# hamaadshah/gan_deeplearning4j

Hardware: NVIDIA H100
Metric: images/sec (full G+D step) (higher is better)
Workload: dtype bf16

## Files before the change

gan_deeplearning4j_b200/_lib.py:

```python
from __future__ import annotations

import ctypes as C
import os

_HERE = os.path.dirname(os.path.abspath(__file__))
LIB_PATH = os.path.join(_HERE, "lib", "libb200gan.so")
NAME_LEN = 64


class B200GanError(RuntimeError):
    def __init__(self, code, msg):
        super().__init__(f"libb200gan error {code}: {msg}")
        self.code = code


class LayerDesc(C.Structure):
    _fields_ = [("type", C.c_int32), ("name", C.c_char * NAME_LEN), ("n_in", C.c_int32), ("n_out", C.c_int32),
                ("k_h", C.c_int32), ("k_w", C.c_int32), ("s_h", C.c_int32), ("s_w", C.c_int32), ("p_h", C.c_int32), ("p_w", C.c_int32),
                ("has_bias", C.c_int32), ("act", C.c_int32), ("act_alpha", C.c_float), ("updater", C.c_int32),
                ("lr", C.c_float), ("beta1", C.c_float), ("beta2", C.c_float), ("eps", C.c_float), ("l2", C.c_float),
                ("bn_decay", C.c_float), ("bn_eps", C.c_float), ("pre_h", C.c_int32), ("pre_w", C.c_int32), ("pre_c", C.c_int32),
                ("loss", C.c_int32), ("frozen", C.c_int32)]


class NetConfig(C.Structure):
    _fields_ = [("in_h", C.c_int32), ("in_w", C.c_int32), ("in_c", C.c_int32), ("max_batch", C.c_int32), ("precision", C.c_int32),
                ("grad_clip", C.c_float), ("xent_clip_eps", C.c_float), ("bn_groups", C.c_int32), ("seed", C.c_uint64)]


class GanConfig(C.Structure):
    _fields_ = [("fake_bn_train", C.c_int32), ("use_cuda_graph", C.c_int32)]


class LrSchedule(C.Structure):
    _fields_ = [("kind", C.c_int32), ("type", C.c_int32), ("initial", C.c_double), ("gamma", C.c_double), ("power", C.c_double),
                ("step", C.c_double), ("decay_rate", C.c_double), ("n_map", C.c_int32), ("map_keys", C.POINTER(C.c_int32)),
                ("map_values", C.POINTER(C.c_double))]


class Constraint(C.Structure):
    _fields_ = [("kind", C.c_int32), ("dims_mask", C.c_int32), ("max_norm", C.c_double), ("min_norm", C.c_double), ("rate", C.c_double)]


class ConvGeom(C.Structure):
    _fields_ = [(k, C.c_int32) for k in ("n", "h", "w", "c", "oh", "ow", "o", "kh", "kw", "sh", "sw", "ph", "pw")]


class TestConvOpts(C.Structure):
    _fields_ = [("epi", C.c_int32), ("act", C.c_int32), ("alpha", C.c_float), ("bias", C.POINTER(C.c_float)), ("scale", C.POINTER(C.c_float)),
                ("groups", C.c_int32), ("aux", C.POINTER(C.c_float)), ("aux2", C.POINTER(C.c_float)), ("stats", C.POINTER(C.c_double)), ("kernel", C.c_char * 64),
                ("bn", C.c_int32), ("max_ctas", C.c_int32), ("poison", C.c_int32), ("w_mn", C.c_int32), ("per_tap", C.c_int32), ("slab", C.c_int32),
                ("defer", C.c_int32), ("db", C.POINTER(C.c_float)), ("param_offset", C.c_int32), ("splits", C.c_int32)]


class EwReduceJob(C.Structure):
    _fields_ = [("n", C.c_int64), ("stride", C.c_int64), ("src_off", C.c_int64), ("dst_off", C.c_int64), ("splits", C.c_int32), ("wide", C.c_int32)]


class TestEwOpts(C.Structure):
    _fields_ = [("op", C.c_int32), ("n", C.c_int64), ("rows", C.c_int32), ("cols", C.c_int32), ("groups", C.c_int32), ("splits", C.c_int32),
                ("stride", C.c_int64)] + [(k, C.c_int32) for k in ("N", "H", "W", "C", "KH", "KW", "SH", "SW", "act")] + [
                ("alpha", C.c_float), ("clip_eps", C.c_float), ("offset", C.c_int32), ("in_place", C.c_int32), ("accumulate", C.c_int32),
                ("poison", C.c_int32), ("n_jobs", C.c_int32), ("jobs", C.POINTER(EwReduceJob)), ("n_seg", C.c_int32),
                ("seg_off", C.POINTER(C.c_int64)), ("seg_len", C.POINTER(C.c_int64)), ("seg_coef", C.POINTER(C.c_float)), ("sumsq", C.c_double),
                ("kernel", C.c_char * 64), ("loss", C.c_int32)]


class TestPoolOpts(C.Structure):
    _fields_ = [("op", C.c_int32), ("pool", C.c_int32), ("pnorm", C.c_float)] + [
                (k, C.c_int32) for k in ("N", "H", "W", "C", "KH", "KW", "SH", "SW", "PH", "PW", "offset", "poison")] + [
                ("kernel", C.c_char * 64), ("splits", C.c_int32)]


_vp, _i32, _i64, _fp = C.c_void_p, C.c_int32, C.c_int64, C.POINTER(C.c_float)
_pvp = C.POINTER(C.c_void_p)

PROTOTYPES = {
    "b2g_version": (_i32, []),
    "b2g_ctx_create": (_i32, [_i32, _pvp]),
    "b2g_ctx_destroy": (_i32, [_vp]),
    "b2g_last_error": (C.c_char_p, []),
    "b2g_sync": (_i32, [_vp]),
    "b2g_launch_count": (_i32, [_vp, C.POINTER(C.c_uint64)]),
    "b2g_timer_start": (_i32, [_vp]),
    "b2g_timer_stop_ms": (_i32, [_vp, _fp]),
    "b2g_flush_l2": (_i32, [_vp]),
    "b2g_device_info": (_i32, [_vp, C.POINTER(_i32), C.POINTER(_i32), C.POINTER(_i32), C.POINTER(C.c_uint64)]),
    "b2g_net_create": (_i32, [_vp, C.POINTER(NetConfig), C.POINTER(LayerDesc), _i32, _pvp]),
    "b2g_net_destroy": (_i32, [_vp]),
    "b2g_net_num_params": (_i32, [_vp, C.POINTER(_i64)]),
    "b2g_net_output_size": (_i32, [_vp, C.POINTER(_i64)]),
    "b2g_net_layer_output_size": (_i32, [_vp, _i32, C.POINTER(_i64)]),
    "b2g_net_set_param": (_i32, [_vp, C.c_char_p, C.c_char_p, _fp, _i64]),
    "b2g_net_get_param": (_i32, [_vp, C.c_char_p, C.c_char_p, _fp, _i64]),
    "b2g_net_get_params": (_i32, [_vp, _fp, _i64]),
    "b2g_net_set_params": (_i32, [_vp, _fp, _i64]),
    "b2g_net_get_gradients": (_i32, [_vp, _fp, _i64]),
    "b2g_net_updater_state_size": (_i32, [_vp, C.POINTER(_i64)]),
    "b2g_net_get_updater_state": (_i32, [_vp, _fp, _i64]),
    "b2g_net_set_updater_state": (_i32, [_vp, _fp, _i64]),
    "b2g_net_output": (_i32, [_vp, _fp, _i32, _i32, _fp]),
    "b2g_net_get_activation": (_i32, [_vp, _i32, _i32, _fp]),
    "b2g_net_compute_gradient_and_score": (_i32, [_vp, _fp, _fp, _i32, _fp]),
    "b2g_net_get_input_gradient": (_i32, [_vp, _i32, _fp]),
    "b2g_net_fit": (_i32, [_vp, _fp, _fp, _i32, _fp]),
    "b2g_net_get_iteration": (_i32, [_vp, C.POINTER(_i64)]),
    "b2g_net_set_iteration": (_i32, [_vp, _i64]),
    "b2g_net_get_dropout_pass": (_i32, [_vp, C.POINTER(_i64)]),
    "b2g_net_set_dropout_pass": (_i32, [_vp, _i64]),
    "b2g_net_set_gradient_normalization": (_i32, [_vp, _i32, C.c_float]),
    "b2g_net_set_lr_schedule": (_i32, [_vp, C.c_char_p, C.POINTER(LrSchedule)]),
    "b2g_net_set_constraints": (_i32, [_vp, C.c_char_p, C.c_char_p, C.POINTER(Constraint), _i32]),
    "b2g_net_apply_constraints": (_i32, [_vp]),
    "b2g_net_get_learning_rate": (_i32, [_vp, C.c_char_p, _fp]),
    "b2g_net_set_dropout_schedule": (_i32, [_vp, C.c_char_p, C.POINTER(LrSchedule)]),
    "b2g_net_get_dropout_value": (_i32, [_vp, C.c_char_p, _fp]),
    "b2g_net_get_epoch": (_i32, [_vp, C.POINTER(_i64)]),
    "b2g_net_set_epoch": (_i32, [_vp, _i64]),
    "b2g_net_simt_gemm_calls": (_i32, [_vp, C.POINTER(C.c_uint64)]),
    "b2g_gan_create": (_i32, [_vp, _vp, C.POINTER(GanConfig), _pvp]),
    "b2g_gan_destroy": (_i32, [_vp]),
    "b2g_gan_step": (_i32, [_vp, _fp, _fp, _fp, _fp, _fp, _fp, _i32, _fp]),
    "b2g_gan_upload": (_i32, [_vp, _fp, _fp, _fp, _fp, _fp, _fp, _i32]),
    "b2g_gan_step_resident": (_i32, [_vp, _i32]),
    "b2g_gan_read_losses": (_i32, [_vp, _fp]),
    "b2g_gan_last_step_ms": (_i32, [_vp, _fp]),
    "b2g_comm_unique_id": (_i32, [_vp]),
    "b2g_ctx_comm_init": (_i32, [_vp, _i32, _i32, _vp]),
    "b2g_ctx_comm_destroy": (_i32, [_vp]),
    "b2g_net_set_grad_allreduce": (_i32, [_vp, _i32]),
    "b2g_net_average_parameters": (_i32, [_vp]),
    "b2g_net_set_sync_bn": (_i32, [_vp, _i32]),
    "b2g_net_set_grad_payload_bf16": (_i32, [_vp, _i32]),
    "b2g_net_enable_p2p_allreduce": (_i32, [_vp, C.POINTER(C.c_int32)]),
    "b2g_ctx_allreduce_test": (_i32, [_vp, _fp, _i64]),
    "b2g_test_conv": (_i32, [_vp, _i32, _i32, _i32, C.POINTER(ConvGeom), _fp, _fp, _fp, _i32, _fp]),
    "b2g_test_hbm_kernels": (_i32, [_vp, _i32, _i32, _i32, _fp]),
    "b2g_test_conv_ex": (_i32, [_vp, _i32, _i32, _i32, C.POINTER(ConvGeom), _fp, _fp, _fp, _i32, _fp, C.POINTER(TestConvOpts)]),
    "b2g_test_bn": (_i32, [_vp, _i32, _i32, _i32, _i32, _i32, _fp, _fp, _fp, _fp, _fp, _fp, _i32, C.c_float, C.c_float, C.c_float,
                           _i32, _fp, _fp, _fp, _fp, _fp, _fp, _fp, _fp]),
    "b2g_test_net_shadow": (_i32, [_vp, _i32, _i32, _fp, _i64]),
    "b2g_test_dropout": (_i32, [_vp, _i32, C.c_uint64, _i32, _i32, _i64, _i32, _i32, _i32, _i32, C.c_float, _fp, _fp, _fp, _fp]),
    "b2g_test_dropout_kind": (_i32, [_vp, _i32, _i32, C.c_uint64, _i32, _i32, _i64, _i32, _i32, _i32, _i32, C.c_float, _fp, _fp, _fp, _fp]),
    "b2g_test_ew": (_i32, [_vp, _i32, C.POINTER(TestEwOpts), _fp, _fp, _fp, _fp, _fp]),
    "b2g_test_pool": (_i32, [_vp, _i32, C.POINTER(TestPoolOpts), _fp, _fp, _fp, _fp, _fp]),
}

_lib = None


def load():
    global _lib
    if _lib is not None:
        return _lib
    if not os.path.exists(LIB_PATH):
        raise B200GanError(-7, f"{LIB_PATH} is missing: build it with `make` (nvcc, sm_90a). There is no CPU fallback.")
    lib = C.CDLL(LIB_PATH, mode=C.RTLD_GLOBAL)
    for name, (res, args) in PROTOTYPES.items():
        fn = getattr(lib, name)
        fn.restype, fn.argtypes = res, args
    _lib = lib
    return lib


def check(code):
    if code != 0:
        raise B200GanError(code, load().b2g_last_error().decode(errors="replace"))
```

gan_deeplearning4j_b200/csrc/engine.cu:

```cuda
#include <cuda_runtime.h>
#include <dlfcn.h>
#include <math.h>
#include <stdarg.h>
#include <stdio.h>
#include <stdlib.h>
#include <string.h>

#include <algorithm>
#include <string>
#include <vector>

#include "../../include/b200gan.h"
#include "kernels.h"

using namespace b2g;

static thread_local char g_err[1024] = "";
static int32_t fail(int32_t code, const char* fmt, ...) {
  va_list ap; va_start(ap, fmt); vsnprintf(g_err, sizeof(g_err), fmt, ap); va_end(ap); return code;
}
#define CU(call) do { cudaError_t e_ = (call); if (e_ != cudaSuccess) return fail(B2G_ERR_CUDA, "%s:%d %s -> %s", __FILE__, __LINE__, #call, cudaGetErrorString(e_)); } while (0)
#define B2(call) do { int32_t r_ = (call); if (r_ != 0) return r_; } while (0)
#define CHECK_KERNELS() CU(cudaGetLastError())

// ... 1553 lines not shown
  if (!n) return fail(B2G_ERR_ARG, "null"); CU(cudaSetDevice(n->ctx->device));
  b2g_net::LayerSched ls; B2(parse_schedule(s, &ls));
  if (layer) { int li = 0; B2(find_dropout_layer(n, layer, &li)); B2(upload_dropout_schedule(n, n->L[li], ls)); }
  else for (auto& l : n->L) if (l.d.type == B2G_LAYER_DROPOUT && !l.d.frozen) B2(upload_dropout_schedule(n, l, ls));
  ++n->settings_gen;
  return 0;
}
extern "C" int32_t b2g_net_get_dropout_value(b2g_net* n, const char* layer, float* out) {
  if (!n || !layer || !out) return fail(B2G_ERR_ARG, "null"); CU(cudaSetDevice(n->ctx->device));
  int li = 0; B2(find_dropout_layer(n, layer, &li));
  const LayerRT& l = n->L[li];
  k_noise_value(l.d.act, l.d.act_alpha, noise_sched(n, l, nullptr, nullptr), n->lr_out, n->ctx->stream); CHECK_KERNELS();
  CU(cudaMemcpyAsync(out, n->lr_out, sizeof(float), cudaMemcpyDeviceToHost, n->ctx->stream)); CU(cudaStreamSynchronize(n->ctx->stream));
  return 0;
}
extern "C" int32_t b2g_net_get_epoch(b2g_net* n, int64_t* out) {
  if (!n || !out) return fail(B2G_ERR_ARG, "null"); CU(cudaSetDevice(n->ctx->device));
  int64_t v = 0; CU(cudaMemcpyAsync(&v, n->epoch_dev, sizeof(v), cudaMemcpyDeviceToHost, n->ctx->stream)); CU(cudaStreamSynchronize(n->ctx->stream)); *out = v; return 0;
}
extern "C" int32_t b2g_net_set_epoch(b2g_net* n, int64_t epoch) {
  if (!n || epoch < 0) return fail(B2G_ERR_ARG, "bad epoch"); CU(cudaSetDevice(n->ctx->device));
  CU(cudaMemcpyAsync(n->epoch_dev, &epoch, sizeof(epoch), cudaMemcpyHostToDevice, n->ctx->stream)); CU(cudaStreamSynchronize(n->ctx->stream)); return 0;
}
extern "C" int32_t b2g_net_simt_gemm_calls(b2g_net* n, uint64_t* out) { if (!n || !out) return fail(B2G_ERR_ARG, "null"); *out = n->simt_gemm_calls; return 0; }

extern "C" int32_t b2g_comm_unique_id(void* id128) { if (!id128) return fail(B2G_ERR_ARG, "null"); B2(nccl_load()); NcclId id; NC(g_nccl.uid(&id)); memcpy(id128, &id, sizeof(id)); return 0; }
extern "C" int32_t b2g_ctx_comm_init(b2g_ctx* c, int32_t world, int32_t rank, const void* id128) {
  if (!c || !id128 || world < 1 || rank < 0 || rank >= world) return fail(B2G_ERR_ARG, "bad communicator arguments");
  B2(nccl_load()); CU(cudaSetDevice(c->device));
  NcclId id; memcpy(&id, id128, sizeof(id));
  NC(g_nccl.init(&c->comm, world, id, rank)); c->world = world; c->rank = rank; return 0;
}
extern "C" int32_t b2g_ctx_comm_destroy(b2g_ctx* c) { if (c && c->comm) { g_nccl.destroy(c->comm); c->comm = nullptr; c->world = 1; c->rank = 0; } return 0; }
extern "C" int32_t b2g_net_set_grad_allreduce(b2g_net* n, int32_t enabled) { if (!n) return fail(B2G_ERR_ARG, "null"); n->grad_allreduce = enabled != 0; return 0; }
extern "C" int32_t b2g_net_set_sync_bn(b2g_net* n, int32_t enabled) { if (!n) return fail(B2G_ERR_ARG, "null"); if (enabled && n->prec != PREC_BF16) return fail(B2G_ERR_UNSUPPORTED, "sync_bn rides on the fused BatchNorm path (BF16 nets)"); n->sync_bn = enabled != 0; return 0; }
extern "C" int32_t b2g_net_set_grad_payload_bf16(b2g_net* n, int32_t enabled) {
  if (!n) return fail(B2G_ERR_ARG, "null"); CU(cudaSetDevice(n->ctx->device));
  if (enabled && !n->ar_buf) B2(dalloc(n, &n->ar_buf, sizeof(__nv_bfloat16) * (size_t)n->n_params));
  n->ar_bf16 = enabled != 0; return 0;
}
extern "C" int32_t b2g_net_enable_p2p_allreduce(b2g_net* n, int32_t* enabled) {
  if (!n) return fail(B2G_ERR_ARG, "null"); b2g_ctx* c = n->ctx; CU(cudaSetDevice(c->device)); if (enabled) *enabled = 0;
  if (!c->comm || c->world < 2) return 0;
  if (c->world > 8 || !g_nccl.ag) return 0;
  cudaStream_t s = c->stream;
  if (!c->p2p_flags) { CU(cudaMalloc(&c->p2p_flags, 16 * sizeof(unsigned))); CU(cudaMalloc(&c->p2p_state, 2 * sizeof(unsigned)));
                       CU(cudaMemsetAsync(c->p2p_flags, 0, 16 * sizeof(unsigned), s)); CU(cudaMemsetAsync(c->p2p_state, 0, 2 * sizeof(unsigned), s)); CU(cudaStreamSynchronize(s)); }
  struct Pair { cudaIpcMemHandle_t flags, grads; };
  Pair mine; memset(&mine, 0, sizeof(mine)); float ok = 1.f;
  if (cudaIpcGetMemHandle(&mine.flags, c->p2p_flags) != cudaSuccess || cudaIpcGetMemHandle(&mine.grads, n->grads) != cudaSuccess) { cudaGetLastError(); ok = 0.f; }
  std::vector<Pair> all(c->world);
  char *d_send = nullptr, *d_recv = nullptr; float* d_ok = nullptr;
  CU(cudaMalloc(&d_send, sizeof(Pair))); CU(cudaMalloc(&d_recv, sizeof(Pair) * c->world)); CU(cudaMalloc(&d_ok, sizeof(float)));
  CU(cudaMemcpyAsync(d_send, &mine, sizeof(Pair), cudaMemcpyHostToDevice, s));
  NC(g_nccl.ag(d_send, d_recv, sizeof(Pair),  0, c->comm, s));
  CU(cudaMemcpyAsync(all.data(), d_recv, sizeof(Pair) * c->world, cudaMemcpyDeviceToHost, s)); CU(cudaStreamSynchronize(s));
  float* pg[8] = {}; unsigned* pf[8] = {};
  for (int r = 0; r < c->world && ok > 0.f; ++r) {
    if (r == c->rank) { pg[r] = n->grads; pf[r] = c->p2p_flags; continue; }
    void* q = nullptr;
    if (cudaIpcOpenMemHandle(&q, all[r].grads, cudaIpcMemLazyEnablePeerAccess) != cudaSuccess) { cudaGetLastError(); ok = 0.f; break; }
    pg[r] = (float*)q;
    if (c->p2p_flags_mapped) pf[r] = c->p2p_peer_flags[r];
    else { if (cudaIpcOpenMemHandle(&q, all[r].flags, cudaIpcMemLazyEnablePeerAccess) != cudaSuccess) { cudaGetLastError(); ok = 0.f; break; } pf[r] = (unsigned*)q; }
  }
  CU(cudaMemcpyAsync(d_ok, &ok, sizeof(float), cudaMemcpyHostToDevice, s)); NC(g_nccl.ar(d_ok, d_ok, 1, 7, 0, c->comm, s));
  float sum = 0.f; CU(cudaMemcpyAsync(&sum, d_ok, sizeof(float), cudaMemcpyDeviceToHost, s)); CU(cudaStreamSynchronize(s));
  cudaFree(d_send); cudaFree(d_recv); cudaFree(d_ok);
  if (sum < (float)c->world - 0.5f) {
    for (int r = 0; r < c->world; ++r) { if (r == c->rank) continue; if (pg[r]) cudaIpcCloseMemHandle(pg[r]); if (!c->p2p_flags_mapped && pf[r]) cudaIpcCloseMemHandle(pf[r]); }
    return 0;
  }
  for (int r = 0; r < c->world; ++r) { n->p2p_peer_grads[r] = pg[r]; c->p2p_peer_flags[r] = pf[r]; }
  c->p2p_flags_mapped = true; n->p2p = true; if (enabled) *enabled = 1;
  return 0;
}
extern "C" int32_t b2g_net_average_parameters(b2g_net* n) {
  if (!n) return fail(B2G_ERR_ARG, "null"); b2g_ctx* c = n->ctx; CU(cudaSetDevice(c->device));
  if (!c->comm || c->world == 1) return 0;
  const float inv = 1.0f / (float)c->world; cudaStream_t s = c->stream;
  float* bufs[4] = {n->params, n->st0, n->st1, n->st2};
  for (float* b : bufs) { if (!b) continue; NC(g_nccl.ar(b, b, (size_t)n->n_params, 7, 0, c->comm, s)); k_scale_f32(b, inv, (size_t)n->n_params, s); }
  net_refresh_shadow(n);
  CU(cudaStreamSynchronize(s)); return 0;
}

namespace {
struct HookMem {
  cudaStream_t s; int prec;
  std::vector<void*> bufs; std::vector<cudaEvent_t> events;
  HookMem(cudaStream_t s_, int prec_) : s(s_), prec(prec_) {}
  HookMem(const HookMem&) = delete; HookMem& operator=(const HookMem&) = delete;
  ~HookMem() { for (void* p : bufs) cudaFree(p); for (cudaEvent_t e : events) cudaEventDestroy(e); }
  int32_t dev(size_t count, size_t es, void** p, size_t off = 0) {
    void* b = nullptr; *p = nullptr; CU(cudaMalloc(&b, es * (count + off) + 16)); bufs.push_back(b); *p = (char*)b + es * off; return 0; }
  int32_t upF(const float* h, size_t count, float** p, size_t off = 0) {
    B2(dev(count, 4, (void**)p, off)); if (h) CU(cudaMemcpyAsync(*p, h, 4 * count, cudaMemcpyHostToDevice, s)); return 0; }
  int32_t toT(const float* f, void* t, size_t count) {
    if (prec == PREC_F32) CU(cudaMemcpyAsync(t, f, 4 * count, cudaMemcpyDeviceToDevice, s)); else k_cast_f32_to_bf16(f, (__nv_bfloat16*)t, count, s); return 0; }
  int32_t upT(const float* h, size_t count, void** p, size_t off = 0) {
    B2(dev(count, prec_size(prec), p, off)); if (!h) return 0;
    if (prec == PREC_F32) { CU(cudaMemcpyAsync(*p, h, 4 * count, cudaMemcpyHostToDevice, s)); return 0; }
    float* f = nullptr; B2(upF(h, count, &f)); return toT(f, *p, count); }
  int32_t downF(float* h, const float* d, size_t count) { if (h) CU(cudaMemcpyAsync(h, d, 4 * count, cudaMemcpyDeviceToHost, s)); return 0; }
  int32_t downT(float* h, const void* d, size_t count) {
    if (!h || prec == PREC_F32) return downF(h, (const float*)d, count);
    float* f = nullptr; B2(upF(nullptr, count, &f)); k_nhwc_to_nchw_f32(prec, d, f, 1, 1, (int)count, s); return downF(h, f, count); }
  int32_t event(cudaEvent_t* e) { CU(cudaEventCreate(e)); events.push_back(*e); return 0; }
};
}

extern "C" int32_t b2g_ctx_allreduce_test(b2g_ctx* c, float* host, int64_t n) {
  if (!c || !host || n < 1) return fail(B2G_ERR_ARG, "null"); if (!c->comm) return fail(B2G_ERR_NCCL, "no communicator"); CU(cudaSetDevice(c->device));
  HookMem m(c->stream, PREC_F32); float* d = nullptr;
  B2(m.upF(host, (size_t)n, &d));
  NC(g_nccl.ar(d, d, (size_t)n, 7, 0, c->comm, c->stream));
  B2(m.downF(host, d, (size_t)n)); CU(cudaStreamSynchronize(c->stream)); return 0;
}

struct TcTestSchedule {
  TcTestSchedule(int bn, int max_ctas, int per_tap, int splits) { g_tc_test_bn = bn; g_tc_test_max_ctas = max_ctas; g_tc_test_per_tap = per_tap; g_tc_test_splits = splits; }
  ~TcTestSchedule() { reset(); }
  void reset() { g_tc_test_bn = 0; g_tc_test_max_ctas = 0; g_tc_test_per_tap = 0; g_tc_test_splits = 0; }
};
enum : unsigned { CO_STATS = 1u << EPI_STATS, CO_BNBWD = 1u << EPI_BNBWD, CO_ACTBWD = 1u << EPI_ACTBWD, CO_BIAS_ACT = 1u << 4, CO_SCALE = 1u << 5,
                  CO_POFF = 1u << 6, CO_BN = 1u << 7, CO_MAX_CTAS = 1u << 8, CO_PER_TAP = 1u << 9, CO_W_MN = 1u << 10, CO_SPLITS = 1u << 11,
                  CO_DEFER = 1u << 12, CO_DB = 1u << 13 };
struct ConvHookImpl {
  const char* kernel;
  bool bf16, tma;
  struct { bool (*shape)(const ConvGeom&); unsigned opts; } kind[3];
};
static bool any_shape(const ConvGeom&) { return true; }
static bool dense_bwd_shape(const ConvGeom& g) { return dense_small_o_supported(g) || dense_small_k_supported(g); }
static bool tc_edge_conv_shape(const ConvGeom& g) { return edge_conv_small_cin_supported(g) && tc_edge_conv_supported(g); }
static bool tc_edge_wgrad_shape(const ConvGeom& g) { return edge_wgrad_small_cin_supported(g) && tc_edge_wgrad_supported(g); }
static const unsigned CO_TC = CO_STATS | CO_BNBWD | CO_ACTBWD | CO_BIAS_ACT | CO_SCALE | CO_BN | CO_MAX_CTAS | CO_PER_TAP;
static const ConvHookImpl kConvHook[6] = {
  {"SIMT kernel", false, false, {{any_shape, CO_BIAS_ACT | CO_SCALE | CO_POFF}, {any_shape, CO_BIAS_ACT | CO_SCALE | CO_POFF}, {any_shape, CO_POFF}}},
  {"tensor-core kernel (BF16, a working tensor-map encoder)", true, true,
   {{tc_fprop_supported, CO_TC | CO_W_MN}, {tc_dgrad_supported, CO_TC}, {tc_wgrad_supported, CO_POFF | CO_SPLITS | CO_DEFER}}},
  {"skinny-layer kernel (<= 4 image channels)", false, false,
   {{edge_conv_small_cin_supported, CO_BIAS_ACT | CO_POFF}, {edge_deconv_small_c_supported, CO_BIAS_ACT | CO_POFF}, {edge_wgrad_small_cin_supported, CO_POFF}}},
  {"skinny-layer tensor-core kernel (BF16, <= 4 image channels, a working tensor-map encoder)", true, true,
   {{tc_edge_conv_shape, CO_BIAS_ACT | CO_MAX_CTAS}, {tc_deconv_ps_supported, CO_ACTBWD | CO_BIAS_ACT | CO_MAX_CTAS},
    {tc_edge_wgrad_shape, CO_POFF | CO_SPLITS | CO_DEFER | CO_DB}}},
  {"dense kernel (1x1 geometry: <= 4 output units, or a short reduction in the input / weight gradient)", false, false,
   {{dense_small_o_supported, CO_BIAS_ACT | CO_POFF}, {dense_bwd_shape, CO_BIAS_ACT | CO_POFF}, {dense_bwd_shape, CO_POFF}}},
  {"few-output conv kernel (BF16, O <= 4, C % 8 == 0, k x k)", true, false,
   {{head_conv_supported, CO_BIAS_ACT | CO_POFF}, {head_conv_supported, CO_BIAS_ACT | CO_POFF}, {head_conv_supported, CO_POFF | CO_SPLITS | CO_DB}}},
};
static constexpr int ik(int impl, int kind) { return 3 * impl + kind; }

extern "C" int32_t b2g_test_conv_ex(b2g_ctx* c, int32_t kind, int32_t impl, int32_t precision, const b2g_conv_geom* gg, const float* a_host, const float* b_host, float* out, int32_t iters, float* ms_per_iter,
                                    b2g_test_conv_opts* opt) {
  if (!c || !gg || !a_host || !b_host || !out) return fail(B2G_ERR_ARG, "null");
  if (kind < 0 || kind > 2 || impl < 0 || impl > 5) return fail(B2G_ERR_ARG, "kind %d / impl %d: kind is 0-2, impl 0-5", kind, impl);
  CU(cudaSetDevice(c->device));
  cudaStream_t s = c->stream; int prec = precision == B2G_PREC_BF16 ? PREC_BF16 : PREC_F32; size_t ts = prec_size(prec);
  ConvGeom g{gg->n, gg->h, gg->w, gg->c, gg->oh, gg->ow, gg->o, gg->kh, gg->kw, gg->sh, gg->sw, gg->ph, gg->pw};
  size_t nx = (size_t)g.N * g.H * g.W * g.C, ny = (size_t)g.N * g.OH * g.OW * g.O, nw = (size_t)g.O * g.KH * g.KW * g.C;
  size_t na = kind == 1 ? ny : nx, nb = kind == 2 ? ny : nw, no = kind == 0 ? ny : kind == 1 ? nx : nw;
  const int oc = kind == 0 ? g.O : g.C;
  const ConvHookImpl& im = kConvHook[impl];
  if ((im.bf16 && prec != PREC_BF16) || (im.tma && !c->tc_ok) || !im.kind[kind].shape(g))
    return fail(B2G_ERR_UNSUPPORTED, "impl %d kind %d: no %s for this shape", impl, kind, im.kernel);
  const b2g_test_conv_opts none{}; const b2g_test_conv_opts& o = opt ? *opt : none;
  const struct { unsigned flag; bool set; const char* what; } asked[] = {
    {o.epi >= EPI_STATS && o.epi <= EPI_ACTBWD ? 1u << o.epi : 1u, o.epi != 0,
     "fused epilogue (epi 1-3: the tensor-core fprop / dgrad, impl 1 kind 0 / 1; epi 3: the pixel-shuffle deconv, impl 3 kind 1)"},
    {CO_BIAS_ACT, o.bias || o.act, "bias / activation (kinds 0 / 1; impl 4 kind 1 on its short-reduction kernel)"},
    {CO_SCALE, o.scale != nullptr, "scale (the SIMT and tensor-core fprop / dgrad, impl 0 / 1 kind 0 / 1)"},
    {CO_POFF, o.param_offset != 0, "param_offset (impl 0 / 2 / 4 / 5, and the tensor-core weight gradients, impl 1 / 3 kind 2)"},
    {CO_BN, o.bn != 0, "bn (the tile width of the tensor-core fprop / dgrad, impl 1 kind 0 / 1)"},
    {CO_MAX_CTAS, o.max_ctas != 0, "max_ctas (a grid cap of tc_conv_kernel and tc_edge_conv_kernel launches, impl 1 / 3 kind 0 / 1)"},
    {CO_PER_TAP, o.per_tap != 0, "per_tap (the tensor-core fprop / dgrad, impl 1 kind 0 / 1)"},
    {CO_W_MN, o.w_mn != 0, "w_mn (the [C][O] weight operand of the 1x1 tensor-core fprop, impl 1 kind 0)"},
    {CO_SPLITS, o.splits != 0, "splits (a forced split count of the weight gradients of impl 1 / 3 / 5)"},
    {CO_DEFER, o.defer != 0, "defer (the tensor-core weight gradients, impl 1 / 3 kind 2)"},
    {CO_DB, o.db != nullptr, "db (the bias column of the edge tensor-core and few-output weight gradients, impl 3 / 5 kind 2)"},
  };
  for (const auto& a : asked) if (a.set && !(im.kind[kind].opts & a.flag)) return fail(B2G_ERR_UNSUPPORTED, "impl %d kind %d takes no %s", impl, kind, a.what);
  if (o.param_offset < 0 || o.max_ctas < 0 || o.splits < 0)
    return fail(B2G_ERR_UNSUPPORTED, "param_offset %d, max_ctas %d, splits %d: none may be negative", o.param_offset, o.max_ctas, o.splits);
  if (o.bn && ((o.bn != 64 && o.bn != 128) || oc % o.bn))
    return fail(B2G_ERR_UNSUPPORTED, "bn %d: the tensor-core fprop / dgrad tile is 64 or 128 columns and must divide the %d output channels", o.bn, oc);
  if (impl == 4 && kind == 1 && (o.bias || o.act) && !dense_small_k_supported(g))
    return fail(B2G_ERR_UNSUPPORTED, "impl 4 kind 1: bias / activation run on the short-reduction kernel only, which has no variant for this shape");
  if (o.w_mn && (g.KH != 1 || g.KW != 1)) return fail(B2G_ERR_UNSUPPORTED, "w_mn: the [C][O] weight operand exists for the 1x1 tensor-core fprop only");
  const bool gemm = impl == 0 || impl == 2 || impl >= 4, tc_wg = kind == 2 && (impl == 1 || impl == 3);
  const int force_splits = o.splits;
  size_t sc = std::max(std::max(std::max(k_simt_wgrad_scratch_floats(g), k_tc_wgrad_scratch_floats(g)), std::max(k_edge_wgrad_scratch_floats(g), k_tc_edge_wgrad_scratch_floats(g))), k_dense_small_o_wgrad_scratch_floats(g)) + 16;
  if (force_splits) sc = std::max(sc, (size_t)force_splits * (impl == 1 || impl == 5 ? nw : (size_t)64 * 16 * g.C + 64) + 16);
  if (impl == 5) sc = std::max(sc, std::max(k_head_wgrad_scratch_floats(g), k_colsum_scratch_floats(g.O)) + 16);
  const size_t woff = (prec == PREC_F32 && kind != 2) ? (size_t)o.param_offset : 0, dwoff = kind == 2 ? (size_t)o.param_offset : 0;
  HookMem m(s, prec);
  float *fa, *fb, *fres, *scratch, *dbres = nullptr, *bias = nullptr, *scale = nullptr; void *ta, *tb, *to; __nv_bfloat16* wps = nullptr;
  B2(m.upF(a_host, na, &fa)); B2(m.upF(b_host, nb, &fb)); B2(m.upF(nullptr, no, &fres, dwoff)); B2(m.upF(nullptr, sc, &scratch));
  B2(m.dev(na, ts, &ta)); B2(m.dev(nb, ts, &tb, woff)); B2(m.dev(no, ts, &to)); B2(m.toT(fa, ta, na)); B2(m.toT(fb, tb, nb));
  if (impl == 3 && kind == 1) { B2(m.dev(k_tc_deconv_ps_weight_elems(g), 2, (void**)&wps)); k_pack_deconv_ps(fb, wps, g.O, g.C, s); }
  if (o.db) B2(m.upF(nullptr, g.O, &dbres, dwoff));
  if (o.bias) B2(m.upF(o.bias, oc, &bias));
  if (o.scale) B2(m.upF(o.scale, oc, &scale));
  const int groups = o.groups > 0 ? o.groups : 1, act = o.act; const float alpha = o.alpha;
  TcEpi epi{}; unsigned long long* d_acc = nullptr;
  epi.mode = o.epi; epi.scale = scale; epi.imgs_per_group = g.N / groups; epi.act = act; epi.alpha = alpha;
  if (o.epi == EPI_STATS || o.epi == EPI_BNBWD) { B2(m.dev(k_bn_acc_elems(oc, groups), 8, (void**)&d_acc)); epi.acc = d_acc; }
  if (o.epi == EPI_BNBWD || o.epi == EPI_ACTBWD) {
    if (!o.aux) return fail(B2G_ERR_ARG, "epilogue %d needs aux", o.epi);
    void* aux = nullptr; B2(m.upT(o.aux, no, &aux)); epi.aux = (const __nv_bfloat16*)aux;
  }
  if (o.epi == EPI_BNBWD) {
    if (!o.aux2) return fail(B2G_ERR_ARG, "epilogue 2 needs aux2 (the BatchNorm input z)");
    void* aux2 = nullptr; B2(m.upT(o.aux2, no, &aux2)); epi.aux2 = (const __nv_bfloat16*)aux2;
  }
  const TcEpi* pe = o.epi || o.scale ? &epi : nullptr;
  const __nv_bfloat16 *ba = (const __nv_bfloat16*)ta, *bb = (const __nv_bfloat16*)tb; __nv_bfloat16* bo = (__nv_bfloat16*)to;
  ReduceList rl{}; ReduceList* prl = o.defer ? &rl : nullptr;
  cudaEvent_t e0, e1; B2(m.event(&e0)); B2(m.event(&e1));
  int reps = iters < 1 ? 1 : iters; int rc = 0, db_written = 0;
  g_tc_last_kernel = ""; g_tc_last_slab = false; g_tc_last_splits = 0; g_gemm_last_kernel = ""; g_gemm_last_splits = 0;
  TcTestSchedule schedule(o.bn, o.max_ctas, o.per_tap != 0, force_splits);
  for (int it = -1; it < reps; ++it) {
    if (it == 0) CU(cudaEventRecord(e0, s));
    if (d_acc) CU(cudaMemsetAsync(d_acc, 0, 8 * k_bn_acc_elems(oc, groups), s));
    if (o.poison) CU(cudaMemsetAsync(to, 0xFF, ts * no, s));
    if (o.poison && kind == 2) { CU(cudaMemsetAsync(fres, 0xFF, 4 * no, s)); CU(cudaMemsetAsync(scratch, 0xFF, 4 * sc, s)); }
    if (o.poison && dbres) CU(cudaMemsetAsync(dbres, 0xFF, 4 * (size_t)g.O, s));
    switch (ik(impl, kind)) {
      case ik(0, 0): k_simt_fprop(prec, prec, g, ta, tb, bias, to, act, alpha, s, scale); break;
      case ik(0, 1): k_simt_dgrad(prec, prec, g, ta, tb, bias, to, act, alpha, s, scale); break;
      case ik(0, 2): k_simt_wgrad(prec, g, ta, tb, fres, scratch, sc, 0, s); break;
      case ik(1, 0): rc = k_tc_fprop(g, ba, bb, bias, bo, act, alpha, s, pe, o.w_mn ? 1 : 0); break;
      case ik(1, 1): rc = k_tc_dgrad(g, ba, bb, bias, bo, act, alpha, s, pe); break;
      case ik(1, 2): rc = k_tc_wgrad(g, ba, bb, fres, scratch, sc, 0, s, prl); break;
      case ik(2, 0): k_edge_conv_small_cin(prec, prec, g, ta, tb, bias, to, act, alpha, s); break;
      case ik(2, 1): k_edge_deconv_small_c(prec, prec, g, ta, tb, bias, to, act, alpha, s); break;
      case ik(2, 2): k_edge_wgrad_small_cin(prec, g, ta, tb, fres, scratch, 0, s); break;
      case ik(3, 0): rc = k_tc_edge_conv(g, ba, bb, bias, bo, act, alpha, s); break;
      case ik(3, 1): rc = k_tc_deconv_ps(g, ba, wps, bias, bo, act, alpha, s, pe); break;
      case ik(3, 2): rc = k_tc_edge_wgrad(g, ba, bb, fres, dbres, scratch, sc, 0, s, prl); if (rc >= 0) { db_written = rc; rc = 0; } break;
      case ik(4, 0): k_dense_small_o_fwd(prec, prec, g, ta, tb, bias, to, act, alpha, s); break;
      case ik(4, 1):
        if (dense_small_o_supported(g) && !bias && !act) k_dense_small_o_dgrad(prec, prec, g, ta, tb, to, s);
        else k_dense_small_k_dgrad(prec, prec, g, ta, tb, bias, to, act, alpha, s);
        break;
      case ik(4, 2): if (dense_small_o_supported(g)) k_dense_small_o_wgrad(prec, g, ta, tb, fres, scratch, 0, s); else k_dense_small_k_wgrad(prec, g, ta, tb, fres, s); break;
      case ik(5, 0): k_head_fwd(g, ba, bb, bias, bo, act, alpha, s); break;
      case ik(5, 1): k_head_dgrad(g, ba, bb, bias, bo, act, alpha, s); break;
      case ik(5, 2): {
        ReduceList hl{};
        if (k_head_wgrad(g, ba, bb, fres, scratch, sc, force_splits, s, &hl)) { rc = -5; break; }
        const int hs = g_gemm_last_splits; k_reduce_multi(hl, s); g_gemm_last_splits = hs;
        if (dbres) { k_colsum(PREC_BF16, tb, g.N * g.OH * g.OW, g.O, scratch, dbres, 0, s); db_written = 1; }
        break;
      }
    }
    if (rc) break;
    if (o.defer) {
      if (!rl.count) { rc = -4; break; }
      k_reduce_multi(rl, s); rl.count = 0;
    }
  }
  schedule.reset();
  CU(cudaEventRecord(e1, s));
  if (rc == -4) return fail(B2G_ERR_CUDA, "defer: the weight gradient queued no reduction");
  if (rc == -5) return fail(B2G_ERR_ARG, "splits %d: the partials do not fit the scratch", force_splits);
  if (rc) return fail(B2G_ERR_CUDA, "tensor-core kernel launch failed (%d)", rc);
  if (opt) {
    strncpy(opt->kernel, gemm ? g_gemm_last_kernel : g_tc_last_kernel, sizeof(opt->kernel) - 1); opt->kernel[sizeof(opt->kernel) - 1] = 0; opt->slab = g_tc_last_slab;
    opt->splits = gemm ? g_gemm_last_splits : tc_wg ? g_tc_last_splits : 0;
  }
  if (o.db) {
    if (!db_written) return fail(B2G_ERR_UNSUPPORTED, "the edge weight gradient produces no bias column for C = %d", g.C);
    B2(m.downF(o.db, dbres, g.O));
  }
  B2(kind == 2 ? m.downF(out, fres, no) : m.downT(out, to, no));
  CU(cudaStreamSynchronize(s)); CHECK_KERNELS();
  if (d_acc && o.stats) {
    std::vector<long long> h(k_bn_acc_elems(oc, groups)); CU(cudaMemcpy(h.data(), d_acc, 8 * h.size(), cudaMemcpyDeviceToHost));
    for (int gi = 0; gi < groups; ++gi) for (int st = 0; st < 2; ++st) for (int ch = 0; ch < oc; ++ch)
      o.stats[((size_t)gi * 2 + st) * oc + ch] = (double)h[((size_t)(gi * 2 + st) * 2 + 0) * oc + ch] / 1024.0 + (double)h[((size_t)(gi * 2 + st) * 2 + 1) * oc + ch] / 1152921504606846976.0;
  }
  float ms = 0.f; CU(cudaEventElapsedTime(&ms, e0, e1)); if (ms_per_iter) *ms_per_iter = ms / reps;
  return 0;
}
extern "C" int32_t b2g_test_conv(b2g_ctx* c, int32_t kind, int32_t impl, int32_t precision, const b2g_conv_geom* gg, const float* a_host, const float* b_host, float* out, int32_t iters, float* ms_per_iter) {
  return b2g_test_conv_ex(c, kind, impl, precision, gg, a_host, b_host, out, iters, ms_per_iter, nullptr);
}

extern "C" int32_t b2g_test_bn(b2g_ctx* c, int32_t precision, int32_t path, int32_t groups, int32_t rows, int32_t C, const float* x, const float* eps_out,
                               const float* gamma, const float* beta, const float* run_mean, const float* run_var, int32_t act, float alpha, float eps, float decay,
                               int32_t want_param_grads, float* y, float* eps_in, float* g_gamma, float* g_beta, float* g_mean, float* g_var, float* mean, float* invstd) {
  if (!c || !x || !eps_out || !gamma || !beta || !run_mean || !run_var || !y || !eps_in || !g_gamma || !g_beta || !g_mean || !g_var || !mean || !invstd) return fail(B2G_ERR_ARG, "null");
  if (groups < 1 || rows < 1 || C < 1 || path < 0 || path > 2) return fail(B2G_ERR_ARG, "bad BatchNorm test arguments");
  const int prec = precision == B2G_PREC_BF16 ? PREC_BF16 : PREC_F32;
  if (path != 0 && !k_bn_vec_ok(prec, C)) return fail(B2G_ERR_UNSUPPORTED, "the accumulator BatchNorm kernels need bf16 and C %% 8 == 0 with 256 %% (C/8) == 0 (C = %d)", C);
  CU(cudaSetDevice(c->device)); cudaStream_t s = c->stream;
  const size_t n = (size_t)groups * rows * C, gc = (size_t)groups * C, ts = prec_size(prec), na = k_bn_acc_elems(C, groups);
  HookMem m(s, prec);
  float *d_gamma, *d_beta, *d_rm, *d_rv, *d_gg, *d_gb, *d_gm, *d_gv, *d_mean, *d_is, *scratch, *coef, *unit; void *tx, *te, *ty, *tei; unsigned long long* acc;
  B2(m.upT(x, n, &tx)); B2(m.upT(eps_out, n, &te)); B2(m.dev(n, ts, &ty)); B2(m.dev(n, ts, &tei));
  B2(m.upF(gamma, C, &d_gamma)); B2(m.upF(beta, C, &d_beta)); B2(m.upF(run_mean, C, &d_rm)); B2(m.upF(run_var, C, &d_rv));
  B2(m.upF(g_gamma, C, &d_gg)); B2(m.upF(g_beta, C, &d_gb)); B2(m.upF(nullptr, C, &d_gm)); B2(m.upF(nullptr, C, &d_gv));
  B2(m.upF(nullptr, gc, &d_mean)); B2(m.upF(nullptr, gc, &d_is)); B2(m.upF(nullptr, k_bn_scratch_floats(C, groups), &scratch));
  B2(m.upF(nullptr, 4 * gc, &coef)); B2(m.upF(nullptr, 4 * gc, &unit)); B2(m.dev(2 * na, 8, (void**)&acc)); CU(cudaMemsetAsync(acc, 0, 8 * 2 * na, s));
  unsigned long long *acc_f = acc, *acc_b = acc + na;
  const int want = want_param_grads ? 1 : 0;
  if (path == 0) {
    k_bn_stats(prec, tx, rows, C, groups, scratch, d_mean, d_is, eps, d_rm, d_rv, d_gm, d_gv, decay, s);
    k_bn_apply(prec, tx, ty, rows, C, groups, d_mean, d_is, d_gamma, d_beta, act, alpha, s);
    k_bn_bwd(prec, tx, te, tei, rows, C, groups, d_mean, d_is, d_gamma, d_beta, act, alpha, scratch, d_gg, d_gb, want, s);
  } else {
    k_bn_stats_acc(tx, rows, C, groups, acc_f, s);
    k_bn_apply_acc(tx, ty, rows, C, groups, acc_f, d_gamma, d_beta, act, alpha, eps, coef, d_rm, d_rv, d_gm, d_gv, decay, s, 1);
    if (path == 1) k_bn_bwd_stats_acc(tx, te, rows, C, groups, coef, act, alpha, acc_b, s);
    else {
      for (int g = 0; g < groups; ++g) for (int k = 0; k < 4; ++k) k_fill_f32(unit + (size_t)(g * 4 + k) * C, (k == 0 || k == 3) ? 1.f : 0.f, C, s);
      k_bn_bwd_stats_acc(tx, te, rows, C, groups, unit, ACT_IDENTITY, 0.f, acc_b, s);
    }
    k_bn_bwd_apply_acc(tx, te, tei, rows, C, groups, coef, act, alpha, path == 2 ? 1 : 0, acc_b, d_gg, d_gb, want, s, 1);
    for (int g = 0; g < groups; ++g) {
      cudaMemcpyAsync(d_mean + (size_t)g * C, coef + (size_t)(g * 4 + 2) * C, 4 * C, cudaMemcpyDeviceToDevice, s);
      cudaMemcpyAsync(d_is + (size_t)g * C, coef + (size_t)(g * 4 + 3) * C, 4 * C, cudaMemcpyDeviceToDevice, s);
    }
  }
  B2(m.downT(y, ty, n)); B2(m.downT(eps_in, tei, n));
  B2(m.downF(g_gamma, d_gg, C)); B2(m.downF(g_beta, d_gb, C)); B2(m.downF(g_mean, d_gm, C)); B2(m.downF(g_var, d_gv, C));
  B2(m.downF(mean, d_mean, gc)); B2(m.downF(invstd, d_is, gc));
  CU(cudaStreamSynchronize(s)); CHECK_KERNELS();
  return 0;
}

extern "C" int32_t b2g_test_dropout(b2g_ctx* c, int32_t precision, uint64_t seed, int32_t layer, int32_t rank, int64_t pass, int32_t rows, int32_t h, int32_t w, int32_t ch,
                                    float p, const float* x, const float* dy, float* y, float* dx) {
  if (!c || !x || !dy || !y || !dx) return fail(B2G_ERR_ARG, "null");
  if (!(p > 0.f && p <= 1.f)) return fail(B2G_ERR_ARG, "dropout retain probability %g outside (0, 1]", (double)p);
  if (rows < 1 || h < 1 || w < 1 || ch < 1 || layer < 0 || layer > 0xffff || rank < 0 || rank > 0xffff || pass < 0) return fail(B2G_ERR_ARG, "bad dropout test arguments");
  const size_t n = (size_t)rows * h * w * ch;
  if (n > 0x7fffffff) return fail(B2G_ERR_UNSUPPORTED, "the dropout test hook takes at most 2^31 - 1 elements (%zu)", n);
  const int prec = precision == B2G_PREC_BF16 ? PREC_BF16 : PREC_F32; const size_t ts = prec_size(prec);
  CU(cudaSetDevice(c->device)); cudaStream_t s = c->stream;
  HookMem m(s, prec);
  void *tx, *te, *ty; uint32_t* mask; unsigned long long* dpass; unsigned* ticket;
  const unsigned long long p0 = (unsigned long long)pass;
  B2(m.upT(x, n, &tx)); B2(m.upT(dy, n, &te)); B2(m.dev(n, ts, &ty)); B2(m.dev((n + 31) / 32, 4, (void**)&mask));
  B2(m.dev(1, sizeof(p0), (void**)&dpass)); B2(m.dev(1, sizeof(unsigned), (void**)&ticket));
  CU(cudaMemcpyAsync(dpass, &p0, sizeof(p0), cudaMemcpyHostToDevice, s)); CU(cudaMemsetAsync(ticket, 0, sizeof(unsigned), s));
  const DropoutArgs a = make_dropout_args(seed, layer, rank, p);
  k_dropout_fwd(prec, tx, ty, mask, n, a, dpass, ticket, 1, s);
  k_dropout_bwd(prec, te, te, mask, n, a.scale, s);
  unsigned long long p1 = 0;
  B2(m.downT(y, ty, n)); B2(m.downT(dx, te, n)); CU(cudaMemcpyAsync(&p1, dpass, sizeof(p1), cudaMemcpyDeviceToHost, s));
  CU(cudaStreamSynchronize(s)); CHECK_KERNELS();
  if (p1 != p0 + 1) return fail(B2G_ERR_CUDA, "dropout test: the forward left the pass counter at %llu, expected %llu", p1, p0 + 1);
  return 0;
}

extern "C" int32_t b2g_test_dropout_kind(b2g_ctx* c, int32_t precision, int32_t kind, uint64_t seed, int32_t layer, int32_t rank, int64_t pass, int32_t rows,
                                         int32_t h, int32_t w, int32_t ch, float v, const float* x, const float* dy, float* y, float* dx) {
  if (!c || !x || !dy || !y || !dx) return fail(B2G_ERR_ARG, "null");
  bool identity = false;
  switch (kind) {
    case B2G_DROPOUT: case B2G_DROPOUT_ALPHA: case B2G_DROPOUT_SPATIAL:
      if (!(v > 0.f && v <= 1.f)) return fail(B2G_ERR_ARG, "dropout retain probability %g outside (0, 1]", (double)v);
      identity = v >= 1.f; break;
    case B2G_DROPOUT_GAUSSIAN_DROPOUT: if (!(v >= 0.f && v < 1.f)) return fail(B2G_ERR_ARG, "GaussianDropout rate %g outside [0, 1)", (double)v); identity = v == 0.f; break;
    case B2G_DROPOUT_GAUSSIAN_NOISE: if (!(v >= 0.f && std::isfinite(v))) return fail(B2G_ERR_ARG, "GaussianNoise stddev %g not finite and >= 0", (double)v); identity = v == 0.f; break;
    default: return fail(B2G_ERR_ARG, "unknown dropout kind %d", kind);
  }
  if (kind == B2G_DROPOUT) return b2g_test_dropout(c, precision, seed, layer, rank, pass, rows, h, w, ch, v, x, dy, y, dx);
  if (rows < 1 || h < 1 || w < 1 || ch < 1 || layer < 0 || layer > 0xffff || rank < 0 || rank > 0xffff || pass < 0) return fail(B2G_ERR_ARG, "bad dropout test arguments");
  const size_t n = (size_t)rows * h * w * ch;
  if (n > 0x7fffffff) return fail(B2G_ERR_UNSUPPORTED, "the dropout test hook takes at most 2^31 - 1 elements (%zu)", n);
// ... 333 lines not shown
```

gan_deeplearning4j_b200/csrc/kernels.h:

```cpp
#pragma once
#include <cuda_runtime.h>
#include <cuda_bf16.h>
#include <math.h>
#include <stdint.h>

namespace b2g {

enum Prec { PREC_F32 = 0, PREC_BF16 = 1 };
enum Act { ACT_IDENTITY = 0, ACT_TANH = 1, ACT_SIGMOID = 2, ACT_RELU = 3, ACT_LRELU = 4,
           ACT_ELU = 5, ACT_SELU = 6, ACT_SOFTPLUS = 7, ACT_SOFTSIGN = 8, ACT_HARDTANH = 9, ACT_HARDSIGMOID = 10, ACT_RELU6 = 11, ACT_SWISH = 12,
           ACT_CUBE = 13, ACT_RATIONALTANH = 14, ACT_RECTIFIEDTANH = 15, ACT_THRESHOLDEDRELU = 16, ACT_EXT_FIRST = ACT_ELU, ACT_EXT_LAST = ACT_THRESHOLDEDRELU };
enum Loss { LOSS_MSE = 2, LOSS_L1 = 3, LOSS_L2 = 4, LOSS_MAE = 5, LOSS_HINGE = 6, LOSS_SQUARED_HINGE = 7, LOSS_WASSERSTEIN = 8 };

inline size_t prec_size(int prec) { return prec == PREC_F32 ? 4 : 2; }

struct ConvGeom {
  int N, H, W, C;
  int OH, OW, O;
  int KH, KW, SH, SW, PH, PW;
};

extern uint64_t g_launch_count;
extern const char* g_ew_last_kernel;
int device_sm_count();
// ... 60 lines not shown
__host__ __device__ inline void noise_derive(int kind, float v, NoiseArgs& a) {
  if (kind == DROP_GAUSSIAN_DROPOUT) { a.scale = (float)sqrt((double)v / (1.0 - (double)v)); return; }
  if (kind == DROP_GAUSSIAN_NOISE) { a.scale = v; return; }
  a.keep_all = v >= 1.f ? 1 : 0; a.threshold = a.keep_all ? 0u : (uint32_t)floor((double)v * 4294967296.0);
  if (kind == DROP_ALPHA) {
    const double ap = -1.0507009873554805 * 1.6732632423543772, p = v, A = 1.0 / sqrt(p + ap * ap * p * (1.0 - p));
    a.scale = (float)A; a.shift = (float)(-A * (1.0 - p) * ap); a.fill = (float)ap;
  } else a.scale = 1.0f / v;
}
struct NoiseRec { unsigned long long P; float v; };
struct UpdSched;
struct NoiseSched { const UpdSched* sched; const int* step; const int64_t* epoch; };
void k_noise_fwd(int prec, int kind, const void* x, void* y, uint32_t* mask, NoiseRec* rec, size_t n, const NoiseArgs& a, const NoiseSched& q,
                 unsigned long long* pass, unsigned* ticket, int bump_pass, cudaStream_t s);
void k_noise_bwd(int prec, int kind, const void* eps_out, void* eps_in, const uint32_t* mask, const NoiseRec* rec, size_t n, const NoiseArgs& a,
                 const NoiseSched& q, cudaStream_t s);
void k_noise_value(int kind, float value, const NoiseSched& q, float* out, cudaStream_t s);

void k_xent(int prec, const void* z, const float* y, void* dz, float* loss_sums, int rows_per_group, int groups, float clip_eps, cudaStream_t s);
void k_sigmoid_out(int prec, const void* z, void* p, size_t n, cudaStream_t s);
void k_softmax_xent(int prec, const void* z, const float* y, void* dz, void* p_out, float* loss_sums, int rows, int K, cudaStream_t s);
int k_loss_blocks(size_t n_per_group, int groups);
void k_loss(int prec, int loss, int act, float alpha, const void* z, const float* y, void* dz, float* loss_sums, int rows_per_group, int n_out, int groups,
            double* partial, unsigned* ticket, cudaStream_t s);
void k_cnn_xent(int prec, const void* z, const float* y, void* dz, float* loss_sums, size_t n_per_group, int groups, float clip_eps, double* partial,
                unsigned* ticket, cudaStream_t s);
int k_cnn_softmax_blocks(int rows_per_group, int groups);
void k_cnn_softmax_xent(int prec, const void* z, const float* y, void* dz, void* p_out, float* loss_sums, int rows_per_group, int C, int groups,
                        double* partial, unsigned* ticket, cudaStream_t s);

enum VertexOp { VERTEX_ADD = 0, VERTEX_SUBTRACT = 1, VERTEX_PRODUCT = 2, VERTEX_AVERAGE = 3, VERTEX_MAX = 4 };
void k_vertex_ew_fwd(int prec, int op, const void* a, const void* b, void* y, size_t n, cudaStream_t s);
void k_vertex_ew_bwd(int prec, int op, int order, void* eps, const void* spine, const void* skip, float* acc, int accumulate, size_t n, cudaStream_t s);
void k_merge_fwd(int prec, const void* a, const void* b, void* y, size_t P, int Ca, int Cb, cudaStream_t s);
void k_merge_bwd(int prec, const void* eps, void* dst, float* acc, size_t P, int Ca, int Cb, int spine_first, int accumulate, cudaStream_t s);
void k_skip_add(int prec, void* eps, const float* acc, size_t n, cudaStream_t s);

void k_colsum(int prec, const void* x, int rows, int C, float* scratch, float* out, int accumulate, cudaStream_t s);
size_t k_colsum_scratch_floats(int C);
void k_sumsq_segments(const float* p, const int64_t* seg_off, const int64_t* seg_len, const float* seg_coef, int nseg, double* out, cudaStream_t s);
void k_reduce_splits(const float* src, float* dst, size_t n, int splits, size_t stride, int accumulate, cudaStream_t s);
struct ReduceJob { const float* src; float* dst; int64_t n, stride; int splits, blocks; };
struct ReduceList { static const int MAX_JOBS = 24; ReduceJob jobs[MAX_JOBS]; int count; };
void reduce_list_push(ReduceList* rl, const float* src, float* dst, int64_t n, int splits, int64_t stride);
void k_reduce_multi(const ReduceList& rl, cudaStream_t s);

struct UpdSeg {
  int64_t off, len;
  int kind;
  float lr, b1, b2, eps;
  float l2;
  float clip;
  int div_mb;
  int64_t off_bf, off_ps;
  int ps_O, ps_C;
};
__device__ __forceinline__ void upd_shadow(const UpdSeg& sg, __nv_bfloat16* __restrict__ shadow, int64_t i, __nv_bfloat16 pb) {
  shadow[sg.off_bf + (i - sg.off)] = pb;
  if (sg.off_ps >= 0) {
    const int e = (int)(i - sg.off), c = e % sg.ps_C, tap = (e / sg.ps_C) % 16, o = e / (sg.ps_C * 16), r = tap >> 2, sx = tap & 3;
    const int py = (r == 0 || r == 2) ? 1 : 0, dyr = r == 3 ? -1 : r == 0 ? 1 : 0, px = (sx == 0 || sx == 2) ? 1 : 0, dxc = sx == 3 ? -1 : sx == 0 ? 1 : 0;
    shadow[sg.off_ps + ((int64_t)((py * 8 + px * 4 + c) * 9 + (dyr + 1) * 3 + (dxc + 1))) * sg.ps_O + o] = pb;
  }
}
struct UpdSched {
  int kind, type;
  int n_map;
  double initial, gamma, power, step, decay;
  const int32_t* keys; const double* vals;
};
void k_updater(float* params, const float* grads, float* st0, float* st1, float* st2, const UpdSeg* segs_dev, const int32_t* chunk_seg_dev,
               const int64_t* chunk_off_dev, int nchunks, float inv_mb, float inv_world, int* step_dev , unsigned* ticket,
               __nv_bfloat16* shadow, const float* gn_mult, const UpdSched* sched, const int64_t* epoch_dev, bool ext, cudaStream_t s);
void k_sched_lr(const UpdSeg* segs_dev, const UpdSched* sched, int seg, const int* step_dev, const int64_t* epoch_dev, float* out, cudaStream_t s);
static const int UPD_CHUNK = 4096;
__device__ inline float sched_lr(const UpdSched& sc, float lr, int it, long long ep) {
  if (sc.kind == 0) return lr;
  const long long ii = sc.type == 1 ? ep : (long long)it;
  const double i = (double)ii;
  double v;
  if (sc.kind == 1) v = sc.initial * pow(sc.gamma, i);
  else if (sc.kind == 2) v = sc.initial / pow(1.0 + sc.gamma * i, sc.power);
  else if (sc.kind == 3) v = sc.initial / (1.0 + exp(-sc.gamma * (i - sc.step)));
  else if (sc.kind == 4) v = sc.initial * pow(sc.decay, floor(i / sc.step));
  else {
    int lo = 0, hi = sc.n_map - 1;
    while (lo < hi) { const int mid = (lo + hi + 1) >> 1; if ((long long)sc.keys[mid] <= ii) lo = mid; else hi = mid - 1; }
    v = sc.vals[lo];
  }
  return (float)v;
}

struct GnGroup { int32_t chunk_begin, chunk_end, seg_begin, seg_end; };
void k_gradnorm(const float* grads, const UpdSeg* segs_dev, const int32_t* chunk_seg_dev, const int64_t* chunk_off_dev, int nchunks,
                const GnGroup* groups_dev, int ngroups, int clip, float threshold, float inv_mb, float inv_world, double* partial, unsigned* ticket,
                float* mult, cudaStream_t s);
enum { CON_ONEPASS = 0, CON_TWOPASS = 1, CON_ELEMWISE = 2 };
static const int CON_CHUNK = 4096, CON_SCHUNK = 256;
struct ConJob {
  UpdSeg sg;
  int kind, path;
  double max_norm, min_norm, rate;
  int K0, R0, K1, R1, K2, groups, R;
  int blk_begin, blocks, blk2_begin, blocks2, chunks;
  int64_t part_begin, mult_begin;
};
void k_constraint_onepass(float* params, __nv_bfloat16* shadow, const ConJob* jobs, int j0, int j1, int blocks, cudaStream_t s);
void k_constraint_twopass(float* params, __nv_bfloat16* shadow, const ConJob* jobs, int j0, int j1, int norm_blocks, int scale_blocks, double* partial,
                          unsigned* ticket, float* mult, cudaStream_t s);
void k_fill_f32(float* p, float v, size_t n, cudaStream_t s);
void k_scale_f32(float* p, float v, size_t n, cudaStream_t s);
struct P2pArgs { float* grads[8]; unsigned* flags[8]; int rank, world; size_t n; unsigned* state; };
void k_p2p_allreduce(const P2pArgs& a, cudaStream_t s);

void k_simt_fprop(int prec, int wprec, const ConvGeom& g, const void* x, const void* w, const float* bias, void* out, int act, float alpha, cudaStream_t s, const float* scale = nullptr);
void k_simt_dgrad(int prec, int wprec, const ConvGeom& g, const void* dy, const void* w, const float* bias, void* dx, int act, float alpha, cudaStream_t s, const float* scale = nullptr);
void k_simt_wgrad(int prec, const ConvGeom& g, const void* x, const void* dy, float* dw, float* scratch, size_t scratch_floats, int accumulate, cudaStream_t s);
size_t k_simt_wgrad_scratch_floats(const ConvGeom& g);
extern const char* g_gemm_last_kernel;
extern int g_gemm_last_splits;

bool edge_deconv_small_c_supported(const ConvGeom& g);
bool edge_conv_small_cin_supported(const ConvGeom& g);
bool edge_wgrad_small_cin_supported(const ConvGeom& g);
bool dense_small_o_supported(const ConvGeom& g);
void k_edge_deconv_small_c(int prec, int wprec, const ConvGeom& g, const void* dy, const void* w, const float* bias, void* dx, int act, float alpha, cudaStream_t s);
void k_edge_conv_small_cin(int prec, int wprec, const ConvGeom& g, const void* x, const void* w, const float* bias, void* out, int act, float alpha, cudaStream_t s);
void k_edge_wgrad_small_cin(int prec, const ConvGeom& g, const void* x, const void* dy, float* dw, float* scratch, int accumulate, cudaStream_t s);
size_t k_edge_wgrad_scratch_floats(const ConvGeom& g);
void k_dense_small_o_fwd(int prec, int wprec, const ConvGeom& g, const void* x, const void* w, const float* bias, void* out, int act, float alpha, cudaStream_t s);
void k_dense_small_o_dgrad(int prec, int wprec, const ConvGeom& g, const void* dy, const void* w, void* dx, cudaStream_t s);
void k_dense_small_o_wgrad(int prec, const ConvGeom& g, const void* x, const void* dy, float* dw, float* scratch, int accumulate, cudaStream_t s);
size_t k_dense_small_o_wgrad_scratch_floats(const ConvGeom& g);
bool dense_small_k_supported(const ConvGeom& g);
void k_dense_small_k_dgrad(int prec, int wprec, const ConvGeom& g, const void* dy, const void* w, const float* bias, void* dx, int act, float alpha, cudaStream_t s);
void k_dense_small_k_wgrad(int prec, const ConvGeom& g, const void* x, const void* dy, float* dw, cudaStream_t s);

bool head_conv_supported(const ConvGeom& g);
size_t k_head_wgrad_scratch_floats(const ConvGeom& g);
void k_head_fwd(const ConvGeom& g, const __nv_bfloat16* x, const __nv_bfloat16* w, const float* bias, __nv_bfloat16* out, int act, float alpha, cudaStream_t s);
void k_head_dgrad(const ConvGeom& g, const __nv_bfloat16* dy, const __nv_bfloat16* w, const float* bias, __nv_bfloat16* dx, int act, float alpha, cudaStream_t s);
int k_head_wgrad(const ConvGeom& g, const __nv_bfloat16* x, const __nv_bfloat16* dy, float* dw, float* part, size_t part_floats, int force_splits, cudaStream_t s,
                 ReduceList* defer);

bool tc_fprop_supported(const ConvGeom& g);
bool tc_dgrad_supported(const ConvGeom& g);
bool tc_wgrad_supported(const ConvGeom& g);
int  tc_init();
extern const char* g_tc_last_kernel;
extern int g_tc_test_bn, g_tc_test_max_ctas;
extern int g_tc_test_per_tap;
extern bool g_tc_last_slab;
extern int g_tc_test_splits, g_tc_last_splits;
enum { EPI_PLAIN = 0, EPI_STATS = 1, EPI_BNBWD = 2, EPI_ACTBWD = 3 };
struct TcEpi {
  int mode;
  const float* scale;
  unsigned long long* acc;
  int imgs_per_group;
  const __nv_bfloat16* aux;
  const __nv_bfloat16* aux2;
  int act; float alpha;
};
int k_tc_fprop(const ConvGeom& g, const __nv_bfloat16* x, const __nv_bfloat16* w, const float* bias, __nv_bfloat16* out, int act, float alpha, cudaStream_t s, const TcEpi* epi = nullptr, int w_mn = 0);
int k_tc_dgrad(const ConvGeom& g, const __nv_bfloat16* dy, const __nv_bfloat16* w, const float* bias, __nv_bfloat16* dx, int act, float alpha, cudaStream_t s, const TcEpi* epi = nullptr);
int k_tc_wgrad(const ConvGeom& g, const __nv_bfloat16* x, const __nv_bfloat16* dy, float* dw, float* scratch, size_t scratch_floats, int accumulate, cudaStream_t s, ReduceList* defer = nullptr);
size_t k_tc_wgrad_scratch_floats(const ConvGeom& g);
bool tc_deconv_ps_shape(const ConvGeom& g);
bool tc_deconv_ps_supported(const ConvGeom& g);
size_t k_tc_deconv_ps_weight_elems(const ConvGeom& g);
void k_pack_deconv_ps(const float* w, __nv_bfloat16* wps, int O, int C, cudaStream_t s);
bool tc_edge_conv_supported(const ConvGeom& g);
bool tc_edge_wgrad_supported(const ConvGeom& g);
size_t k_tc_edge_wgrad_scratch_floats(const ConvGeom& g);
int k_tc_edge_conv(const ConvGeom& g, const __nv_bfloat16* x, const __nv_bfloat16* w, const float* bias, __nv_bfloat16* out, int act, float alpha, cudaStream_t s);
int k_tc_edge_wgrad(const ConvGeom& g, const __nv_bfloat16* x, const __nv_bfloat16* dy, float* dw, float* db, float* scratch, size_t scratch_floats, int accumulate, cudaStream_t s, ReduceList* defer = nullptr);
int k_tc_deconv_ps(const ConvGeom& g, const __nv_bfloat16* dy, const __nv_bfloat16* wps, const float* bias, __nv_bfloat16* dx, int act, float alpha, cudaStream_t s, const TcEpi* epi = nullptr);

}
```

gan_deeplearning4j_b200/csrc/kernels_tc.cu:

```cuda
#include <cuda.h>
#include <stdio.h>
#include <stdlib.h>
#include <algorithm>

#include "common.cuh"
#include "kernels.h"

namespace b2g {

typedef CUresult (*PFN_encodeTiled)(CUtensorMap*, CUtensorMapDataType, cuuint32_t, void*, const cuuint64_t*, const cuuint64_t*, const cuuint32_t*,
                                    const cuuint32_t*, CUtensorMapInterleave, CUtensorMapSwizzle, CUtensorMapL2promotion, CUtensorMapFloatOOBfill);
static PFN_encodeTiled g_encode = nullptr;

int tc_init() {
  if (g_encode) return 0;
  void* fn = nullptr; cudaDriverEntryPointQueryResult q;
  if (cudaGetDriverEntryPoint("cuTensorMapEncodeTiled", &fn, cudaEnableDefault, &q) != cudaSuccess || !fn || q != cudaDriverEntryPointSuccess) return -1;
  g_encode = (PFN_encodeTiled)fn; return 0;
}

static int make_map_bf16(CUtensorMap* m, const void* base, int rank, const cuuint64_t* dims, const cuuint64_t* strides_bytes, const cuuint32_t* box, const cuuint32_t* estr) {
  if (!g_encode) return -1;
  CUresult r = g_encode(m, CU_TENSOR_MAP_DATA_TYPE_BFLOAT16, (cuuint32_t)rank, const_cast<void*>(base), dims, strides_bytes, box, estr, CU_TENSOR_MAP_INTERLEAVE_NONE,
                        CU_TENSOR_MAP_SWIZZLE_128B, CU_TENSOR_MAP_L2_PROMOTION_L2_256B, CU_TENSOR_MAP_FLOAT_OOB_FILL_NONE);
  if (r != CUDA_SUCCESS) { fprintf(stderr, "[b200gan] cuTensorMapEncodeTiled failed: %d (rank %d)\n", (int)r, rank); return -1; }
  return 0;
}

__device__ __forceinline__ uint32_t smem_u32(const void* p) { return (uint32_t)__cvta_generic_to_shared(p); }
__device__ __forceinline__ void mbar_init(uint32_t bar, uint32_t count) { asm volatile("mbarrier.init.shared::cta.b64 [%0], %1;" ::"r"(bar), "r"(count)); }
__device__ __forceinline__ void fence_mbar_init() { asm volatile("fence.mbarrier_init.release.cluster;" ::: "memory"); }
__device__ __forceinline__ void mbar_expect_tx(uint32_t bar, uint32_t bytes) { asm volatile("mbarrier.arrive.expect_tx.shared::cta.b64 _, [%0], %1;" ::"r"(bar), "r"(bytes) : "memory"); }
__device__ __forceinline__ void mbar_arrive(uint32_t bar) { asm volatile("mbarrier.arrive.shared::cta.b64 _, [%0];" ::"r"(bar) : "memory"); }
__device__ int g_tc_timeout_flag = 0;
__device__ __forceinline__ void mbar_wait(uint32_t bar, uint32_t parity) {
  uint32_t done = 0;
  for (uint32_t it = 0; it < (1u << 26); ++it) {
    asm volatile("{\n\t.reg .pred p;\n\tmbarrier.try_wait.parity.shared::cta.b64 p, [%1], %2;\n\tselp.u32 %0, 1, 0, p;\n\t}" : "=r"(done) : "r"(bar), "r"(parity) : "memory");
    if (done) return;
  }
  g_tc_timeout_flag = 1; __trap();
}
__device__ __forceinline__ void tma_load_4d(uint32_t dst, const CUtensorMap* map, uint32_t bar, int c0, int c1, int c2, int c3) {
  asm volatile("cp.async.bulk.tensor.4d.shared::cluster.global.tile.mbarrier::complete_tx::bytes [%0], [%1, {%3, %4, %5, %6}], [%2];"
               ::"r"(dst), "l"(map), "r"(bar), "r"(c0), "r"(c1), "r"(c2), "r"(c3) : "memory");
}
__device__ __forceinline__ void tma_load_3d(uint32_t dst, const CUtensorMap* map, uint32_t bar, int c0, int c1, int c2) {
  asm volatile("cp.async.bulk.tensor.3d.shared::cluster.global.tile.mbarrier::complete_tx::bytes [%0], [%1, {%3, %4, %5}], [%2];"
               ::"r"(dst), "l"(map), "r"(bar), "r"(c0), "r"(c1), "r"(c2) : "memory");
}
__device__ __forceinline__ void tma_load_2d(uint32_t dst, const CUtensorMap* map, uint32_t bar, int c0, int c1) {
  asm volatile("cp.async.bulk.tensor.2d.shared::cluster.global.tile.mbarrier::complete_tx::bytes [%0], [%1, {%3, %4}], [%2];"
               ::"r"(dst), "l"(map), "r"(bar), "r"(c0), "r"(c1) : "memory");
}
__device__ __forceinline__ bool elect_one_sync() {
  uint32_t pred = 0;
  asm volatile("{\n\t.reg .pred P1;\n\t.reg .b32 rx;\n\telect.sync rx|P1, %1;\n\t@P1 mov.s32 %0, 1;\n\t}" : "+r"(pred) : "r"(0xffffffffu));
  return pred != 0;
}
__device__ __forceinline__ void prefetch_map(const CUtensorMap* map) { asm volatile("prefetch.tensormap [%0];" ::"l"(map) : "memory"); }
__device__ __forceinline__ void fence_proxy_async_smem() { asm volatile("fence.proxy.async.shared::cta;" ::: "memory"); }

__device__ __forceinline__ uint64_t gmma_desc(uint32_t saddr, uint32_t lbo_bytes) {
  return (uint64_t)((saddr & 0x3FFFFu) >> 4) | ((uint64_t)((lbo_bytes >> 4) & 0x3FFF) << 16) | ((uint64_t)(1024 >> 4) << 32) | (1ull << 62);
}
__device__ __forceinline__ uint64_t desc_kmajor_sw128(uint32_t saddr) { return gmma_desc(saddr, 16); }
__device__ __forceinline__ uint64_t desc_mnmajor_sw128(uint32_t saddr, uint32_t lbo_bytes) { return gmma_desc(saddr, lbo_bytes); }

__device__ __forceinline__ void wg_fence() { asm volatile("wgmma.fence.sync.aligned;" ::: "memory"); }
__device__ __forceinline__ void wg_commit() { asm volatile("wgmma.commit_group.sync.aligned;" ::: "memory"); }
template <int N>
__device__ __forceinline__ void wg_wait() { asm volatile("wgmma.wait_group.sync.aligned %0;" ::"n"(N) : "memory"); }

template <int TA, int TB>
__device__ __forceinline__ void wgmma_n64(float (&d)[32], uint64_t da, uint64_t db) {
  asm volatile(
      "wgmma.mma_async.sync.aligned.m64n64k16.f32.bf16.bf16 "
      "{%0, %1, %2, %3, %4, %5, %6, %7, %8, %9, %10, %11, %12, %13, %14, %15, %16, %17, %18, %19, %20, %21, %22, %23, %24, %25, %26, %27, %28, %29, %30, %31}, "
      "%32, %33, 1, 1, 1, %34, %35;"
      : "+f"(d[0]), "+f"(d[1]), "+f"(d[2]), "+f"(d[3]), "+f"(d[4]), "+f"(d[5]), "+f"(d[6]), "+f"(d[7]), "+f"(d[8]), "+f"(d[9]), "+f"(d[10]),
        "+f"(d[11]), "+f"(d[12]), "+f"(d[13]), "+f"(d[14]), "+f"(d[15]), "+f"(d[16]), "+f"(d[17]), "+f"(d[18]), "+f"(d[19]), "+f"(d[20]),
        "+f"(d[21]), "+f"(d[22]), "+f"(d[23]), "+f"(d[24]), "+f"(d[25]), "+f"(d[26]), "+f"(d[27]), "+f"(d[28]), "+f"(d[29]), "+f"(d[30]), "+f"(d[31])
      : "l"(da), "l"(db), "n"(TA), "n"(TB));
}
template <int TA, int TB>
__device__ __forceinline__ void wgmma_n128(float (&d0)[32], float (&d1)[32], uint64_t da, uint64_t db) {
  asm volatile(
      "wgmma.mma_async.sync.aligned.m64n128k16.f32.bf16.bf16 "
      "{%0, %1, %2, %3, %4, %5, %6, %7, %8, %9, %10, %11, %12, %13, %14, %15, %16, %17, %18, %19, %20, %21, %22, %23, %24, %25, %26, %27, %28, %29, %30, %31, %32, %33, %34, %35, %36, %37, %38, %39, %40, %41, %42, %43, %44, %45, %46, %47, %48, %49, %50, %51, %52, %53, %54, %55, %56, %57, %58, %59, %60, %61, %62, %63}, "
      "%64, %65, 1, 1, 1, %66, %67;"
      : "+f"(d0[0]), "+f"(d0[1]), "+f"(d0[2]), "+f"(d0[3]), "+f"(d0[4]), "+f"(d0[5]), "+f"(d0[6]), "+f"(d0[7]), "+f"(d0[8]), "+f"(d0[9]), "+f"(d0[10]), "+f"(d0[11]), "+f"(d0[12]), "+f"(d0[13]), "+f"(d0[14]), "+f"(d0[15]), "+f"(d0[16]), "+f"(d0[17]), "+f"(d0[18]), "+f"(d0[19]), "+f"(d0[20]), "+f"(d0[21]), "+f"(d0[22]), "+f"(d0[23]), "+f"(d0[24]), "+f"(d0[25]), "+f"(d0[26]), "+f"(d0[27]), "+f"(d0[28]), "+f"(d0[29]), "+f"(d0[30]), "+f"(d0[31]),
        "+f"(d1[0]), "+f"(d1[1]), "+f"(d1[2]), "+f"(d1[3]), "+f"(d1[4]), "+f"(d1[5]), "+f"(d1[6]), "+f"(d1[7]), "+f"(d1[8]), "+f"(d1[9]), "+f"(d1[10]), "+f"(d1[11]), "+f"(d1[12]), "+f"(d1[13]), "+f"(d1[14]), "+f"(d1[15]), "+f"(d1[16]), "+f"(d1[17]), "+f"(d1[18]), "+f"(d1[19]), "+f"(d1[20]), "+f"(d1[21]), "+f"(d1[22]), "+f"(d1[23]), "+f"(d1[24]), "+f"(d1[25]), "+f"(d1[26]), "+f"(d1[27]), "+f"(d1[28]), "+f"(d1[29]), "+f"(d1[30]), "+f"(d1[31])
      : "l"(da), "l"(db), "n"(TA), "n"(TB));
}
__device__ __forceinline__ void wgmma_n16(float (&d)[8], uint64_t da, uint64_t db) {
  asm volatile(
      "wgmma.mma_async.sync.aligned.m64n16k16.f32.bf16.bf16 {%0, %1, %2, %3, %4, %5, %6, %7}, %8, %9, 1, 1, 1, 0, 0;"
      : "+f"(d[0]), "+f"(d[1]), "+f"(d[2]), "+f"(d[3]), "+f"(d[4]), "+f"(d[5]), "+f"(d[6]), "+f"(d[7])
      : "l"(da), "l"(db));
}



struct TcConvParams {
  int mode;
  int Nt, Ht, Wt;
  int GH, GW;
  int tiles_y;
  int taps_h, taps_w;
  int slab_bytes;
  int a_wg_bytes;
  int a_tap_bytes;
  int chunks;
  int KW, SH, SW, PH, PW;
  int OC;
  int outH, outW;
  int b_mn;
  const float* bias; const float* scale; int act; float alpha;
  __nv_bfloat16* out;
  int epi;
  unsigned long long* acc;
  int imgs_per_group;
  const __nv_bfloat16* aux;
  const __nv_bfloat16* aux2;
  int tiles_m, tiles_n, phases;
};

static constexpr int TC_THREADS = 384;
static constexpr int TC_CONV_THREADS = 640;
static constexpr int SLAB_ROWS = 144;
template <int BN, int STAGES, int EPI = EPI_PLAIN, bool SLAB = false>
struct TcSmem {
  static constexpr int A_BYTES = (SLAB ? SLAB_ROWS : 128) * 128;
  static constexpr int B_BYTES = (SLAB ? 2 : 1) * BN * 128;
  static constexpr int STAGE_BYTES = A_BYTES + B_BYTES;
  static constexpr int RING_BYTES = STAGES * STAGE_BYTES;
  static constexpr int ACC_PITCH = BN + 4;
  static constexpr int PARK_BYTES = 128 * ACC_PITCH * 4;
  static constexpr int PARKS = BN >= 128 ? 1 : 2;
  static constexpr int PARK_OFF = RING_BYTES;
  static constexpr int BAR_OFF = PARK_OFF + PARKS * PARK_BYTES;
  static constexpr int STAT_OFF = BAR_OFF + 256;
  static constexpr int STG_OFF = STAT_OFF + ((EPI == EPI_STATS || EPI == EPI_BNBWD) ? 4 * 2 * BN * 4 : 0);
  static constexpr int TOTAL = STG_OFF + (BN >= 32 ? 8 * 2048 : 0) + 1024;
  static_assert(TOTAL <= 227 * 1024, "one CTA per SM must fit the shared memory of an sm_90 SM");
};

__device__ __forceinline__ void epi_bar_sync() { asm volatile("bar.sync 1, 256;" ::: "memory"); }
template <int N> __device__ __forceinline__ void setmaxnreg_inc() { asm volatile("setmaxnreg.inc.sync.aligned.u32 %0;" ::"n"(N)); }
template <int N> __device__ __forceinline__ void setmaxnreg_dec() { asm volatile("setmaxnreg.dec.sync.aligned.u32 %0;" ::"n"(N)); }

template <int OFF>
__device__ __forceinline__ void warp_colsum_level(float (&a)[32], int lane) {
  const bool up = (lane & OFF) != 0;
#pragma unroll
  for (int j = 0; j < OFF; ++j) {
    const float lo = a[j], hi = a[j + OFF];
    const float send = up ? lo : hi, keep = up ? hi : lo;
    a[j] = keep + __shfl_xor_sync(0xffffffffu, send, OFF);
  }
  if constexpr (OFF > 1) warp_colsum_level<OFF / 2>(a, lane);
}
__device__ __forceinline__ void warp_colsum32(float (&a)[32], int lane) { warp_colsum_level<16>(a, lane); }

template <int BN, int EPI, bool AFFINE>
__device__ __forceinline__ void epi_tile(const TcConvParams& p, const float* srow, size_t roff, int nb0, int group, float* sst, uint4* stg, int q, int lane, int ep_tid,
                                         int c_beg, int c_end) {
  constexpr bool stats = EPI == EPI_STATS || EPI == EPI_BNBWD;
  const bool has_bias = p.bias != nullptr;
  const int sub = lane >> 2, cq = lane & 3, sx = (lane >> 1) & 3;
  size_t roff_i[4];
#pragma unroll
  for (int i = 0; i < 4; ++i) roff_i[i] = __shfl_sync(0xffffffffu, (unsigned long long)roff, i * 8 + sub) + cq * 8;
#pragma unroll 1
  for (int c0 = c_beg; c0 < c_end; c0 += 32) {
    uint32_t v[32];
    uint4 gy[4], gz[4], ax[4], az[4];
    if constexpr (EPI >= EPI_BNBWD) {
#pragma unroll
      for (int i = 0; i < 4; ++i) gy[i] = *reinterpret_cast<const uint4*>(p.aux + roff_i[i] + c0);
    }
    if constexpr (EPI == EPI_BNBWD) {
#pragma unroll
      for (int i = 0; i < 4; ++i) gz[i] = *reinterpret_cast<const uint4*>(p.aux2 + roff_i[i] + c0);
    }
    if constexpr (EPI >= EPI_BNBWD) {
#pragma unroll
      for (int i = 0; i < 4; ++i) { const int r = i * 8 + sub; stg[r * 4 + (cq ^ ((r >> 1) & 3))] = gy[i]; }
      __syncwarp();
#pragma unroll
      for (int j = 0; j < 4; ++j) ax[j] = stg[lane * 4 + (j ^ sx)];
      __syncwarp();
    }
    if constexpr (EPI == EPI_BNBWD) {
#pragma unroll
      for (int i = 0; i < 4; ++i) { const int r = i * 8 + sub; stg[r * 4 + (cq ^ ((r >> 1) & 3))] = gz[i]; }
      __syncwarp();
#pragma unroll
      for (int j = 0; j < 4; ++j) az[j] = stg[lane * 4 + (j ^ sx)];
      __syncwarp();
    }
#pragma unroll
    for (int j = 0; j < 8; ++j) { const uint4 t = reinterpret_cast<const uint4*>(srow + c0)[j]; v[4 * j] = t.x; v[4 * j + 1] = t.y; v[4 * j + 2] = t.z; v[4 * j + 3] = t.w; }
    float o[32], s2[32];
    if constexpr (EPI == EPI_BNBWD) {
      const __nv_bfloat162* yb = reinterpret_cast<const __nv_bfloat162*>(ax);
      const __nv_bfloat162* zb = reinterpret_cast<const __nv_bfloat162*>(az);
#define B2G_BNBWD_LOOP(ACTC)                                                                                                   \
  _Pragma("unroll") for (int j = 0; j < 16; ++j) {                                                                             \
    const float2 y2 = __bfloat1622float2(yb[j]), z2 = __bfloat1622float2(zb[j]);                                               \
    o[2 * j] = __uint_as_float(v[2 * j]) * act_grad_from_out(ACTC, y2.x, p.alpha);                                             \
    o[2 * j + 1] = __uint_as_float(v[2 * j + 1]) * act_grad_from_out(ACTC, y2.y, p.alpha);                                     \
    s2[2 * j] = z2.x; s2[2 * j + 1] = z2.y;                                                                                    \
  }
      if (p.act == ACT_LRELU) { B2G_BNBWD_LOOP(ACT_LRELU) }
      else if (p.act == ACT_RELU) { B2G_BNBWD_LOOP(ACT_RELU) }
      else { B2G_BNBWD_LOOP(p.act) }
#undef B2G_BNBWD_LOOP
    } else if constexpr (EPI == EPI_ACTBWD) {
      const __nv_bfloat162* ab = reinterpret_cast<const __nv_bfloat162*>(ax);
#define B2G_ACTBWD_LOOP(ACTC)                                                                                                  \
  _Pragma("unroll") for (int j = 0; j < 16; ++j) {                                                                             \
    const float2 a2 = __bfloat1622float2(ab[j]);                                                                               \
    o[2 * j] = __uint_as_float(v[2 * j]) * act_grad_from_out(ACTC, a2.x, p.alpha);                                             \
    o[2 * j + 1] = __uint_as_float(v[2 * j + 1]) * act_grad_from_out(ACTC, a2.y, p.alpha);                                     \
  }
      if (p.act == ACT_LRELU) { B2G_ACTBWD_LOOP(ACT_LRELU) }
      else if (p.act == ACT_TANH) { B2G_ACTBWD_LOOP(ACT_TANH) }
      else { B2G_ACTBWD_LOOP(p.act) }
#undef B2G_ACTBWD_LOOP
    } else {
#define B2G_EPI_LOOP(ACTC)                                                                                                     \
  _Pragma("unroll") for (int j = 0; j < 32; ++j) {                                                                             \
    float a = __uint_as_float(v[j]);                                                                                           \
    if (AFFINE) a = fmaf(a, p.scale[nb0 + c0 + j], p.bias[nb0 + c0 + j]);                                                      \
    else if (has_bias) a += p.bias[nb0 + c0 + j];                                                                              \
    o[j] = act_fwd(ACTC, a, p.alpha);                                                                                          \
  }
      if (p.act == ACT_IDENTITY) { B2G_EPI_LOOP(ACT_IDENTITY) }
      else if (p.act == ACT_LRELU) { B2G_EPI_LOOP(ACT_LRELU) }
      else if (p.act == ACT_RELU) { B2G_EPI_LOOP(ACT_RELU) }
      else { B2G_EPI_LOOP(p.act) }
#undef B2G_EPI_LOOP
    }
    uint32_t packed[16];
#pragma unroll
    for (int j = 0; j < 16; ++j) {
      __nv_bfloat162 h = __floats2bfloat162_rn(o[2 * j], o[2 * j + 1]);
      packed[j] = *reinterpret_cast<uint32_t*>(&h);
      if constexpr (stats) { const float2 r = __bfloat1622float2(h); o[2 * j] = r.x; o[2 * j + 1] = r.y; }
    }
#pragma unroll
    for (int j = 0; j < 4; ++j) stg[lane * 4 + (j ^ sx)] = make_uint4(packed[4 * j], packed[4 * j + 1], packed[4 * j + 2], packed[4 * j + 3]);
    __syncwarp();
#pragma unroll
    for (int i = 0; i < 4; ++i) { const int r = i * 8 + sub; *reinterpret_cast<uint4*>(p.out + roff_i[i] + c0) = stg[r * 4 + (cq ^ ((r >> 1) & 3))]; }
    __syncwarp();
    if constexpr (stats) {
      if constexpr (EPI == EPI_STATS) {
#pragma unroll
        for (int j = 0; j < 32; ++j) s2[j] = o[j] * o[j];
      } else {
#pragma unroll
        for (int j = 0; j < 32; ++j) s2[j] = o[j] * s2[j];
      }
      warp_colsum32(o, lane); warp_colsum32(s2, lane);
      sst[(q * 2 + 0) * BN + c0 + lane] = o[0];
      sst[(q * 2 + 1) * BN + c0 + lane] = s2[0];
    }
  }
  if constexpr (stats) {
    epi_bar_sync();
    for (int col = ep_tid; col < BN; col += 256) {
#pragma unroll
      for (int st = 0; st < 2; ++st) {
        const float s = ((sst[(0 * 2 + st) * BN + col] + sst[(1 * 2 + st) * BN + col]) + sst[(2 * 2 + st) * BN + col]) + sst[(3 * 2 + st) * BN + col];
        sacc_add(p.acc + (size_t)(group * 2 + st) * 2 * p.OC, (size_t)p.OC, (size_t)(nb0 + col), s);
      }
    }
  }
}

template <int BN>
__device__ __forceinline__ void load_b_tile(const TcConvParams& p, const CUtensorMap* tmB, uint32_t dst, uint32_t bar, int ch, int wtap, int nb0) {
  if (!p.b_mn) tma_load_3d(dst, tmB, bar, ch * 64, wtap, nb0);
  else {
#pragma unroll
    for (int j = 0; j < (BN >= 64 ? BN / 64 : 1); ++j) tma_load_3d(dst + j * 8192, tmB, bar, nb0 + j * 64, wtap, ch * 64);
  }
}
template <int BN, int NB, int NACC>
__device__ __forceinline__ void mma_kblock(float (&acc)[NB][NACC], uint32_t a_smem, uint32_t b_smem, int b_mn) {
  const uint64_t adesc = desc_kmajor_sw128(a_smem);
  if constexpr (BN < 64) {
    const uint64_t bdesc = desc_kmajor_sw128(b_smem);
#pragma unroll
    for (int k = 0; k < 4; ++k) wgmma_n16(acc[0], adesc + 2 * k, bdesc + 2 * k);
  } else if constexpr (NB == 2) {
    if (!b_mn) {
#pragma unroll
      for (int k = 0; k < 4; ++k) wgmma_n128<0, 0>(acc[0], acc[1], adesc + 2 * k, desc_kmajor_sw128(b_smem) + 2 * k);
    } else {
#pragma unroll
      for (int k = 0; k < 4; ++k) wgmma_n128<0, 1>(acc[0], acc[1], adesc + 2 * k, desc_mnmajor_sw128(b_smem + k * 2048, 8192));
    }
  } else if (!b_mn) {
#pragma unroll
    for (int k = 0; k < 4; ++k) wgmma_n64<0, 0>(acc[0], adesc + 2 * k, desc_kmajor_sw128(b_smem) + 2 * k);
  } else {
#pragma unroll
    for (int k = 0; k < 4; ++k) wgmma_n64<0, 1>(acc[0], adesc + 2 * k, desc_mnmajor_sw128(b_smem + k * 2048, 8192));
  }
}
__device__ __forceinline__ void tap_coords(const TcConvParams& p, int ta, int tb, int py, int px, int& ax, int& dy_, int& wtap) {
  if (p.mode == 0) { dy_ = -p.PH + ta; ax = -p.PW + tb; wtap = ta * p.KW + tb; }
  else {
    const int r = py == 0 ? (ta == 0 ? 1 : 3) : (ta == 0 ? 0 : 2), dyr = py == 0 ? (ta == 0 ? 0 : -1) : (ta == 0 ? 1 : 0);
    const int sx = px == 0 ? (tb == 0 ? 1 : 3) : (tb == 0 ? 0 : 2), dxc = px == 0 ? (tb == 0 ? 0 : -1) : (tb == 0 ? 1 : 0);
    dy_ = dyr; ax = dxc; wtap = r * 4 + sx;
  }
}
__device__ __forceinline__ void slab_coords(const TcConvParams& p, int ta, int tb, int py, int px, int& ax, int& dy_, int& wlo, int& whi) {
  int ax2, dy2;
  tap_coords(p, p.mode == 0 ? ta : 1, tb, py, px, ax, dy_, wlo);
  tap_coords(p, p.mode == 0 ? ta + 2 : 0, tb, py, px, ax2, dy2, whi);
}

template <int BN>
struct TcConvRegs {
  static constexpr int LAUNCH = 96, PRODUCER = 24, MMA = BN >= 128 ? 96 : 64, EPI = BN >= 128 ? 128 : 160;
  static_assert(PRODUCER + 2 * MMA + 2 * EPI <= 5 * LAUNCH, "setmaxnreg budget exceeds the launch allocation");
};
template <int BN, int STAGES, int EPI, bool AFFINE, bool PS = false, bool SLAB = false>
__global__ void __launch_bounds__(TC_CONV_THREADS, 1) tc_conv_kernel(const __grid_constant__ CUtensorMap tmA, const __grid_constant__ CUtensorMap tmB, const TcConvParams p) {
  using S = TcSmem<BN, STAGES, EPI, SLAB>;
  using R = TcConvRegs<BN>;
  constexpr int NB = BN >= 64 ? BN / 64 : 1, NACC = BN >= 64 ? 32 : BN / 2;
  extern __shared__ uint8_t smem_raw[];
  const uint32_t smem_base = (smem_u32(smem_raw) + 1023u) & ~1023u;
  uint8_t* smem_gen = smem_raw + (smem_base - smem_u32(smem_raw));
  const uint32_t bar_full = smem_base + S::BAR_OFF;
  const uint32_t bar_empty = bar_full + 8 * STAGES;
  const uint32_t park_full = bar_empty + 8 * STAGES;
  const uint32_t park_empty = park_full + 8 * S::PARKS;
  float* sst = reinterpret_cast<float*>(smem_gen + S::STAT_OFF);
  const int warp = threadIdx.x >> 5, lane = threadIdx.x & 31;
  const int num_kb = p.taps_h * p.taps_w * p.chunks;
  const int tiles = p.tiles_m * p.tiles_n * p.phases;
  auto tile_coords = [&](int t, int& nb0, int& phase, int& n0, int& y0) {
    const int mt = t % p.tiles_m, r = t / p.tiles_m;
    nb0 = (r % p.tiles_n) * BN; phase = r / p.tiles_n;
    if (p.Nt > 1) { n0 = mt * p.Nt; y0 = 0; } else { n0 = mt / p.tiles_y; y0 = (mt % p.tiles_y) * p.Ht; }
  };

  if (threadIdx.x == 0) {
    prefetch_map(&tmA); prefetch_map(&tmB);
    for (int s = 0; s < STAGES; ++s) { mbar_init(bar_full + 8 * s, 1); mbar_init(bar_empty + 8 * s, 8); }
    for (int k = 0; k < S::PARKS; ++k) { mbar_init(park_full + 8 * k, 256); mbar_init(park_empty + 8 * k, 256); }
    fence_mbar_init();
  }
  __syncthreads();
  pdl_wait();

  if (warp >= 16) {
    setmaxnreg_dec<R::PRODUCER>();
    if (warp == 16) {
      int s = 0; uint32_t ph = 0;
      for (int t = blockIdx.x; t < tiles; t += gridDim.x) {
        int nb0, phase, n0, y0; tile_coords(t, nb0, phase, n0, y0);
        const int py = phase >> 1, px = phase & 1;
        const int ybase = p.mode == 0 ? y0 * p.SH : y0;
        int ch = 0, ta = 0, tb = 0;
        int ax, dy_, wtap, wtap2 = 0;
        auto coords = [&]() { if constexpr (SLAB) slab_coords(p, ta, tb, py, px, ax, dy_, wtap, wtap2); else tap_coords(p, ta, tb, py, px, ax, dy_, wtap); };
        coords();
        for (int kb = 0; kb < num_kb; ++kb) {
          mbar_wait(bar_empty + 8 * s, ph ^ 1);
          if (elect_one_sync()) {
            const uint32_t st = smem_base + s * S::STAGE_BYTES;
            mbar_expect_tx(bar_full + 8 * s, SLAB ? p.slab_bytes + S::B_BYTES : S::STAGE_BYTES);
            tma_load_4d(st, &tmA, bar_full + 8 * s, ch * 64, ax, ybase + dy_, n0);
            load_b_tile<BN>(p, &tmB, st + S::A_BYTES, bar_full + 8 * s, ch, wtap, nb0);
            if constexpr (SLAB) load_b_tile<BN>(p, &tmB, st + S::A_BYTES + BN * 128, bar_full + 8 * s, ch, wtap2, nb0);
          }
          __syncwarp();
          if (++s == STAGES) { s = 0; ph ^= 1; }
          if (++ch == p.chunks) { ch = 0; if (++tb == p.taps_w) { tb = 0; ++ta; } coords(); }
        }
      }
    }
  } else if (warp < 8) {
    if constexpr (R::MMA < R::LAUNCH) setmaxnreg_dec<R::MMA>();
    const int wg = warp >> 2;
    const int r0 = wg * 64 + (warp & 3) * 16 + (lane >> 2);
    int s = 0, k = 0; uint32_t ph = 0, kph = 0;
    for (int t = blockIdx.x; t < tiles; t += gridDim.x) {
      float acc[NB][NACC];
#pragma unroll
      for (int nb = 0; nb < NB; ++nb)
#pragma unroll
        for (int j = 0; j < NACC; ++j) acc[nb][j] = 0.f;
      int prev = -1;
      for (int kb = 0; kb < num_kb; ++kb) {
        mbar_wait(bar_full + 8 * s, ph);
        wg_fence();
        const uint32_t st = smem_base + s * S::STAGE_BYTES;
        if constexpr (SLAB) {
          const uint32_t a = st + wg * p.a_wg_bytes;
          mma_kblock<BN, NB, NACC>(acc, a, st + S::A_BYTES, p.b_mn);
          mma_kblock<BN, NB, NACC>(acc, a + p.a_tap_bytes, st + S::A_BYTES + BN * 128, p.b_mn);
        } else {
          mma_kblock<BN, NB, NACC>(acc, st + wg * 8192, st + S::A_BYTES, PS ? 0 : p.b_mn);
        }
        wg_commit();
        wg_wait<1>();
        if (prev >= 0 && lane == 0) mbar_arrive(bar_empty + 8 * prev);
        prev = s;
        if (++s == STAGES) { s = 0; ph ^= 1; }
      }
      wg_wait<0>();
      if (lane == 0) mbar_arrive(bar_empty + 8 * prev);
      mbar_wait(park_empty + 8 * k, kph ^ 1);
      float* park = reinterpret_cast<float*>(smem_gen + S::PARK_OFF + k * S::PARK_BYTES);
#pragma unroll
      for (int nb = 0; nb < NB; ++nb)
#pragma unroll
        for (int j = 0; j < NACC / 4; ++j) {
          const int col = nb * 64 + j * 8 + 2 * (lane & 3);
          *reinterpret_cast<float2*>(park + r0 * S::ACC_PITCH + col) = make_float2(acc[nb][4 * j], acc[nb][4 * j + 1]);
          *reinterpret_cast<float2*>(park + (r0 + 8) * S::ACC_PITCH + col) = make_float2(acc[nb][4 * j + 2], acc[nb][4 * j + 3]);
        }
      mbar_arrive(park_full + 8 * k);
      if (++k == S::PARKS) { k = 0; kph ^= 1; }
    }
  } else {
    setmaxnreg_inc<R::EPI>();
    const int ew = warp - 8, q = ew & 3, half = ew >> 2;
    const int row = q * 32 + lane;
    const int img = row / (p.Ht * p.Wt), rem = row % (p.Ht * p.Wt), yy = rem / p.Wt, xx = rem % p.Wt;
    int k = 0; uint32_t kph = 0;
    for (int t = blockIdx.x; t < tiles; t += gridDim.x) {
      int nb0, phase, n0, y0; tile_coords(t, nb0, phase, n0, y0);
      const int py = phase >> 1, px = phase & 1;
      const int n = n0 + img, gy = y0 + yy, gx = xx;
      mbar_wait(park_full + 8 * k, kph);
      const float* srow = reinterpret_cast<const float*>(smem_gen + S::PARK_OFF + k * S::PARK_BYTES) + row * S::ACC_PITCH;
      if constexpr (PS) {
        if (half == 0) {
          const int C = p.OC;
#pragma unroll
          for (int ppy = 0; ppy < 2; ++ppy) {
            const size_t doff = (((size_t)n * p.outH + 2 * gy + ppy) * p.outW + 2 * gx) * C;
            __nv_bfloat16* dst = p.out + doff;
            float o[8];
#pragma unroll
            for (int ppx = 0; ppx < 2; ++ppx)
#pragma unroll
              for (int c = 0; c < 4; ++c) {
                float a = srow[(ppy * 2 + ppx) * 4 + c];
                if constexpr (EPI == EPI_ACTBWD) { if (c < C) a *= act_grad_from_out(p.act, __bfloat162float(p.aux[doff + ppx * C + c]), p.alpha); }
                else { if (p.bias && c < C) a += p.bias[c]; a = act_fwd(p.act, a, p.alpha); }
                o[ppx * 4 + c] = a;
              }
            if (C == 3) {
              __nv_bfloat162 h0 = __floats2bfloat162_rn(o[0], o[1]), h1 = __floats2bfloat162_rn(o[2], o[4]), h2 = __floats2bfloat162_rn(o[5], o[6]);
              uint32_t* d32 = reinterpret_cast<uint32_t*>(dst);
              d32[0] = *reinterpret_cast<uint32_t*>(&h0); d32[1] = *reinterpret_cast<uint32_t*>(&h1); d32[2] = *reinterpret_cast<uint32_t*>(&h2);
            } else {
#pragma unroll
              for (int ppx = 0; ppx < 2; ++ppx)
#pragma unroll
                for (int c = 0; c < 4; ++c) if (c < C) dst[ppx * C + c] = __float2bfloat16(o[ppx * 4 + c]);
            }
          }
        }
      } else {
        size_t pix;
        if (p.mode == 0) pix = ((size_t)n * p.outH + gy) * p.outW + gx;
        else pix = ((size_t)n * p.outH + 2 * gy + py) * p.outW + 2 * gx + px;
        const int group = p.imgs_per_group > 0 ? n0 / p.imgs_per_group : 0;
        epi_tile<BN, EPI, AFFINE>(p, srow, pix * p.OC + nb0, nb0, group, sst, reinterpret_cast<uint4*>(smem_gen + S::STG_OFF) + ew * 128, q, lane,
                                  (int)threadIdx.x - 256, half * (BN / 2), (half + 1) * (BN / 2));
        if constexpr (EPI == EPI_STATS || EPI == EPI_BNBWD) epi_bar_sync();
      }
      mbar_arrive(park_empty + 8 * k);
      if (++k == S::PARKS) { k = 0; kph ^= 1; }
    }
  }
}

const char* g_tc_last_kernel = "";
bool g_tc_last_slab = false;
int g_tc_test_bn = 0, g_tc_test_max_ctas = 0, g_tc_test_per_tap = 0, g_tc_test_splits = 0;
int g_tc_last_splits = 0;
static int tc_device() { int dev = 0; cudaGetDevice(&dev); return dev < 0 || dev >= 64 ? 0 : dev; }
#define TC_SET_SMEM_ONCE(kernel, bytes)                                                                                            \
  do { static bool set_[64] = {}; const int d_ = tc_device();                                                                       \
       if (!set_[d_]) { if (cudaFuncSetAttribute(kernel, cudaFuncAttributeMaxDynamicSharedMemorySize, (int)(bytes)) != cudaSuccess) return -2; set_[d_] = true; } } while (0)

static bool pick_row_tile(int N, int GH, int GW, int rows, int* Nt, int* Ht, int* Wt) {
  const int P = GH * GW;
  if (GW > rows || rows % GW) return false;
  if (P >= rows) { if (P % rows) return false; *Nt = 1; *Ht = rows / GW; *Wt = GW; return GH % *Ht == 0; }
  if (rows % P || N % (rows / P)) return false;
  *Nt = rows / P; *Ht = GH; *Wt = GW; return true;
}
static int pick_bn(int OC) { return OC % 128 == 0 ? 128 : OC % 64 == 0 ? 64 : 0; }
static int pick_bn_fill(int OC, long m_tiles_x_phases) {
  if (g_tc_test_bn) return g_tc_test_bn;
  const int target = device_sm_count();
  int bn = pick_bn(OC);
  while (bn > 64 && m_tiles_x_phases * (OC / bn) < target) bn /= 2;
  return bn;
}

bool tc_fprop_supported(const ConvGeom& g) {
  int a, b, c;
  return g.C % 64 == 0 && pick_bn(g.O) != 0 && g.SH >= 1 && g.SH <= 2 && g.SW == g.SH && g.KH * g.KW * (g.C / 64) >= 1 &&
         pick_row_tile(g.N, g.OH, g.OW, 128, &a, &b, &c) && c * g.SW <= 256 && b * g.SH <= 256 && g.N >= 1;
}
bool tc_dgrad_supported(const ConvGeom& g) {
  int a, b, c;
  return g.KH == 4 && g.KW == 4 && g.SH == 2 && g.SW == 2 && g.PH == 1 && g.PW == 1 && g.O % 64 == 0 && pick_bn(g.C) != 0 && g.H == 2 * g.OH && g.W == 2 * g.OW &&
         pick_row_tile(g.N, g.OH, g.OW, 128, &a, &b, &c);
}
static bool tc_epi_ok(const TcEpi* e, int Nt) { return !e || e->mode == EPI_PLAIN || e->mode == EPI_ACTBWD || (e->imgs_per_group > 0 && e->imgs_per_group % Nt == 0 && e->acc); }

template <int BN, int STAGES, int EPI, bool AFFINE, bool PS = false, bool SLAB = false>
static int launch_conv_e(const CUtensorMap& tmA, const CUtensorMap& tmB, const TcConvParams& p, cudaStream_t s) {
  using S = TcSmem<BN, STAGES, EPI, SLAB>;
  TC_SET_SMEM_ONCE((tc_conv_kernel<BN, STAGES, EPI, AFFINE, PS, SLAB>), S::TOTAL);
  const long tiles = (long)p.tiles_m * p.tiles_n * p.phases;
  const unsigned grid = (unsigned)std::min<long>(tiles, g_tc_test_max_ctas > 0 ? g_tc_test_max_ctas : device_sm_count());
  launch_pdl(tc_conv_kernel<BN, STAGES, EPI, AFFINE, PS, SLAB>, dim3(grid), dim3(TC_CONV_THREADS), (size_t)(S::TOTAL), s, tmA, tmB, p);
  LAUNCHED();
  return cudaPeekAtLastError() == cudaSuccess ? 0 : -3;
}
template <int BN, int STAGES, bool SLAB>
static int launch_conv(const CUtensorMap& tmA, const CUtensorMap& tmB, const TcConvParams& p, cudaStream_t s, const char* name) {
  g_tc_last_kernel = name; g_tc_last_slab = SLAB;
  switch (p.epi) {
    case EPI_STATS: return launch_conv_e<BN, STAGES, EPI_STATS, false, false, SLAB>(tmA, tmB, p, s);
    case EPI_BNBWD: return launch_conv_e<BN, STAGES, EPI_BNBWD, false, false, SLAB>(tmA, tmB, p, s);
    case EPI_ACTBWD: return launch_conv_e<BN, STAGES, EPI_ACTBWD, false, false, SLAB>(tmA, tmB, p, s);
  }
  return (p.scale && p.bias) ? launch_conv_e<BN, STAGES, EPI_PLAIN, true, false, SLAB>(tmA, tmB, p, s) : launch_conv_e<BN, STAGES, EPI_PLAIN, false, false, SLAB>(tmA, tmB, p, s);
}
static int dispatch_conv(int BN, bool slab, const CUtensorMap& tmA, const CUtensorMap& tmB, const TcConvParams& p, cudaStream_t s) {
  switch (BN * 2 + slab) {
    case 128: return launch_conv<64, 4, false>(tmA, tmB, p, s, "tc_conv_kernel<64,4>");
    case 256: return launch_conv<128, 4, false>(tmA, tmB, p, s, "tc_conv_kernel<128,4>");
    case 129: return launch_conv<64, 4, true>(tmA, tmB, p, s, "tc_conv_kernel<64,4>");
  }
  return -4;
}
static bool slab_tile(const TcConvParams& p, int BN) {
  if (g_tc_test_per_tap || BN != 64 || p.Wt % 8) return false;
  if (!((p.Nt == 1 && p.Ht >= 2) || (p.Nt == 2 && p.Ht * p.Wt == 64))) return false;
  return p.Nt * (p.Ht + 1) * p.Wt <= SLAB_ROWS;
}
static bool is_k4s2p1_geom(const ConvGeom& g) { return g.KH == 4 && g.KW == 4 && g.SH == 2 && g.SW == 2 && g.PH == 1 && g.PW == 1 && g.H == 2 * g.OH && g.W == 2 * g.OW; }
static void set_slab(TcConvParams& p) {
  p.taps_h = p.mode == 0 ? 2 : 1;
  p.slab_bytes = p.Nt * (p.Ht + 1) * p.Wt * 128;
  p.a_wg_bytes = p.Nt == 1 ? 64 * 128 : (p.Ht + 1) * p.Wt * 128;
  p.a_tap_bytes = p.Wt * 128;
}

static int weight_map(CUtensorMap* m, const __nv_bfloat16* w, int rows, int taps, int inner, int box_rows) {
  cuuint64_t dims[3] = {(cuuint64_t)inner, (cuuint64_t)taps, (cuuint64_t)rows};
  cuuint64_t strides[2] = {(cuuint64_t)inner * 2, (cuuint64_t)taps * inner * 2};
  cuuint32_t box[3] = {64, 1, (cuuint32_t)box_rows}; cuuint32_t es[3] = {1, 1, 1};
  return make_map_bf16(m, w, 3, dims, strides, box, es);
}
static void fill_epi(TcConvParams& p, const float* bias, int act, float alpha, const TcEpi* e) {
  p.bias = bias; p.act = act; p.alpha = alpha; p.epi = EPI_PLAIN;
  if (!e) return;
  p.scale = e->scale; p.epi = e->mode; p.acc = e->acc; p.imgs_per_group = e->mode == EPI_STATS || e->mode == EPI_BNBWD ? e->imgs_per_group : 0;
  p.aux = e->aux; p.aux2 = e->aux2;
  if (e->mode == EPI_BNBWD || e->mode == EPI_ACTBWD) { p.act = e->act; p.alpha = e->alpha; p.bias = nullptr; p.scale = nullptr; }
}

int k_tc_fprop(const ConvGeom& g, const __nv_bfloat16* x, const __nv_bfloat16* w, const float* bias, __nv_bfloat16* out, int act, float alpha, cudaStream_t s, const TcEpi* epi, int w_mn) {
  TcConvParams p{}; p.mode = 0;
  if (!pick_row_tile(g.N, g.OH, g.OW, 128, &p.Nt, &p.Ht, &p.Wt) || !tc_epi_ok(epi, p.Nt)) return -1;
  if (w_mn && (g.KH != 1 || g.KW != 1)) return -1;
  const int BN = pick_bn_fill(g.O, (long)g.N * g.OH * g.OW / 128);
  p.GH = g.OH; p.GW = g.OW; p.tiles_y = g.OH / p.Ht; p.taps_h = g.KH; p.taps_w = g.KW; p.chunks = g.C / 64; p.KW = g.KW;
  p.SH = g.SH; p.SW = g.SW; p.PH = g.PH; p.PW = g.PW; p.OC = g.O; p.outH = g.OH; p.outW = g.OW; p.out = out; p.b_mn = w_mn;
  fill_epi(p, bias, act, alpha, epi);
  const bool slab = is_k4s2p1_geom(g) && !w_mn && slab_tile(p, BN);
  if (slab) set_slab(p);
  CUtensorMap tmA, tmB;
  cuuint64_t dims[4] = {(cuuint64_t)g.C, (cuuint64_t)g.W, (cuuint64_t)g.H, (cuuint64_t)g.N};
  cuuint64_t strides[3] = {(cuuint64_t)g.C * 2, (cuuint64_t)g.W * g.C * 2, (cuuint64_t)g.H * g.W * g.C * 2};
  cuuint32_t box[4] = {64, (cuuint32_t)(p.Wt * g.SW), (cuuint32_t)((p.Ht + slab) * g.SH), (cuuint32_t)p.Nt};
  cuuint32_t es[4] = {1, (cuuint32_t)g.SW, (cuuint32_t)g.SH, 1};
  if (make_map_bf16(&tmA, x, 4, dims, strides, box, es)) return -1;
  p.tiles_m = g.N * g.OH * g.OW / 128; p.tiles_n = g.O / BN; p.phases = 1;
  if (w_mn ? weight_map(&tmB, w, g.C, 1, g.O, 64) : weight_map(&tmB, w, g.O, g.KH * g.KW, g.C, BN)) return -1;
  return dispatch_conv(BN, slab, tmA, tmB, p, s);
}

int k_tc_dgrad(const ConvGeom& g, const __nv_bfloat16* dy, const __nv_bfloat16* w, const float* bias, __nv_bfloat16* dx, int act, float alpha, cudaStream_t s, const TcEpi* epi) {
  TcConvParams p{}; p.mode = 1;
  if (!pick_row_tile(g.N, g.OH, g.OW, 128, &p.Nt, &p.Ht, &p.Wt) || !tc_epi_ok(epi, p.Nt)) return -1;
  const int BN = pick_bn_fill(g.C, (long)g.N * g.OH * g.OW / 128 * 4);
  p.GH = g.OH; p.GW = g.OW; p.tiles_y = g.OH / p.Ht; p.taps_h = 2; p.taps_w = 2; p.chunks = g.O / 64; p.KW = 4;
  p.SH = 1; p.SW = 1; p.PH = 0; p.PW = 0; p.OC = g.C; p.outH = g.H; p.outW = g.W; p.out = dx; p.b_mn = 1;
  fill_epi(p, bias, act, alpha, epi);
  const bool slab = slab_tile(p, BN);
  if (slab) set_slab(p);
  CUtensorMap tmA, tmB;
  cuuint64_t dims[4] = {(cuuint64_t)g.O, (cuuint64_t)g.OW, (cuuint64_t)g.OH, (cuuint64_t)g.N};
  cuuint64_t strides[3] = {(cuuint64_t)g.O * 2, (cuuint64_t)g.OW * g.O * 2, (cuuint64_t)g.OH * g.OW * g.O * 2};
  cuuint32_t box[4] = {64, (cuuint32_t)p.Wt, (cuuint32_t)(p.Ht + slab), (cuuint32_t)p.Nt};
  cuuint32_t es[4] = {1, 1, 1, 1};
  if (weight_map(&tmB, w, g.O, 16, g.C, 64)) return -1;
  if (make_map_bf16(&tmA, dy, 4, dims, strides, box, es)) return -1;
  p.tiles_m = g.N * g.OH * g.OW / 128; p.tiles_n = g.C / BN; p.phases = 4;
  return dispatch_conv(BN, slab, tmA, tmB, p, s);
}

bool tc_deconv_ps_shape(const ConvGeom& g) { return is_k4s2p1_geom(g) && g.C >= 1 && g.C <= 4 && g.O % 64 == 0; }
bool tc_deconv_ps_supported(const ConvGeom& g) { int a, b, c; return tc_deconv_ps_shape(g) && pick_row_tile(g.N, g.OH, g.OW, 128, &a, &b, &c); }
size_t k_tc_deconv_ps_weight_elems(const ConvGeom& g) { return tc_deconv_ps_shape(g) ? (size_t)16 * 9 * g.O : 0; }
__global__ void pack_deconv_ps_kernel(const float* __restrict__ w, __nv_bfloat16* __restrict__ wps, int O, int C) { pdl_wait();
  const int idx = blockIdx.x * blockDim.x + threadIdx.x; if (idx >= 16 * 9 * O) return;
  const int o = idx % O, t = (idx / O) % 9, n = idx / (9 * O);
  const int py = n >> 3, px = (n >> 2) & 1, c = n & 3, dyr = t / 3 - 1, dxc = t % 3 - 1;
  const int r = dyr == -1 ? (py == 0 ? 3 : -1) : dyr == 0 ? (py == 0 ? 1 : 2) : (py == 1 ? 0 : -1);
  const int sx = dxc == -1 ? (px == 0 ? 3 : -1) : dxc == 0 ? (px == 0 ? 1 : 2) : (px == 1 ? 0 : -1);
  wps[idx] = __float2bfloat16((r >= 0 && sx >= 0 && c < C) ? w[((size_t)o * 16 + r * 4 + sx) * C + c] : 0.f);
}
void k_pack_deconv_ps(const float* w, __nv_bfloat16* wps, int O, int C, cudaStream_t s) {
  launch_pdl(pack_deconv_ps_kernel, dim3((16 * 9 * O + 255) / 256), dim3(256), (size_t)(0), s, w, wps, O, C); LAUNCHED();
}
int k_tc_deconv_ps(const ConvGeom& g, const __nv_bfloat16* dy, const __nv_bfloat16* wps, const float* bias, __nv_bfloat16* dx, int act, float alpha, cudaStream_t s, const TcEpi* epi) {
  TcConvParams p{}; p.mode = 0;
  if (!tc_deconv_ps_shape(g) || !pick_row_tile(g.N, g.OH, g.OW, 128, &p.Nt, &p.Ht, &p.Wt)) return -1;
  if (epi && epi->mode != EPI_PLAIN && epi->mode != EPI_ACTBWD) return -1;
  p.GH = g.OH; p.GW = g.OW; p.tiles_y = g.OH / p.Ht; p.taps_h = 3; p.taps_w = 3; p.chunks = g.O / 64; p.KW = 3;
  p.SH = 1; p.SW = 1; p.PH = 1; p.PW = 1; p.OC = g.C; p.outH = g.H; p.outW = g.W; p.out = dx;
  fill_epi(p, bias, act, alpha, epi);
  CUtensorMap tmA, tmB;
  cuuint64_t dims[4] = {(cuuint64_t)g.O, (cuuint64_t)g.OW, (cuuint64_t)g.OH, (cuuint64_t)g.N};
  cuuint64_t strides[3] = {(cuuint64_t)g.O * 2, (cuuint64_t)g.OW * g.O * 2, (cuuint64_t)g.OH * g.OW * g.O * 2};
  cuuint32_t box[4] = {64, (cuuint32_t)p.Wt, (cuuint32_t)p.Ht, (cuuint32_t)p.Nt}; cuuint32_t es[4] = {1, 1, 1, 1};
  if (make_map_bf16(&tmA, dy, 4, dims, strides, box, es)) return -1;
  if (weight_map(&tmB, wps, 16, 9, g.O, 16)) return -1;
  p.tiles_m = (int)((long)g.N * g.OH * g.OW / 128); p.tiles_n = 1; p.phases = 1;
  g_tc_last_kernel = "tc_conv_kernel<16,4,PS>";
  return p.epi == EPI_ACTBWD ? launch_conv_e<16, 4, EPI_ACTBWD, false, true>(tmA, tmB, p, s) : launch_conv_e<16, 4, EPI_PLAIN, false, true>(tmA, tmB, p, s);
}

struct TcEdgeParams {
  const __nv_bfloat16* x; const __nv_bfloat16* w; const __nv_bfloat16* dy; const float* bias; __nv_bfloat16* out; float* part; float* part_b;
  int N, H, W, C, OH, OW, O, Ht, tiles_y, tiles_total, tiles_per_cta, act; float alpha;
};
static constexpr int EDGE_SLAB_BYTES = 6144;
__device__ __forceinline__ uint32_t swz128(int row, int byte) { return (uint32_t)(row * 128 + ((((byte >> 4) ^ (row & 7)) << 4) | (byte & 15))); }

struct EdgeSlabRegs { uint4 v[3]; };
__device__ __forceinline__ void edge_fetch_slab(const TcEdgeParams& p, int n, int oy0, EdgeSlabRegs& r) {
  const int WC = p.W * p.C, cpr = WC >> 3, total = (2 * p.Ht + 2) * cpr;
#pragma unroll
  for (int q = 0; q < 3; ++q) {
    const int i = threadIdx.x + q * 128; r.v[q] = make_uint4(0u, 0u, 0u, 0u);
    if (i < total) { const int j = i / cpr, cc = i - j * cpr, iy = 2 * oy0 - 1 + j;
      if (iy >= 0 && iy < p.H) r.v[q] = __ldg(reinterpret_cast<const uint4*>(p.x + ((size_t)n * p.H + iy) * WC) + cc); }
  }
}
__device__ __forceinline__ void edge_store_slab(const TcEdgeParams& p, const EdgeSlabRegs& r, uint8_t* slab) {
  const int total = (2 * p.Ht + 2) * ((p.W * p.C) >> 3);
#pragma unroll
  for (int q = 0; q < 3; ++q) { const int i = threadIdx.x + q * 128; if (i < total) reinterpret_cast<uint4*>(slab)[i] = r.v[q]; }
}
template <int C>
__device__ __forceinline__ void edge_build_row_c(const TcEdgeParams& p, const uint8_t* slab, uint8_t* tile, int row, bool ones) {
  const int WC = p.W * C, oy_l = row / p.OW, ox = row - oy_l * p.OW;
  const int lo = ox == 0 ? C : 0, hi = ox == p.OW - 1 ? 3 * C : 4 * C;
  uint32_t out[32];
#pragma unroll
  for (int i = 0; i < 32; ++i) out[i] = 0u;
#pragma unroll
  for (int r = 0; r < 4; ++r) {
    const int b0 = ((2 * oy_l + r) * WC + (2 * ox - 1) * C) * 2;
    if (C & 1) {
      const uint32_t* wp = reinterpret_cast<const uint32_t*>(slab + b0 - 2);
      uint32_t w[2 * C + 1];
#pragma unroll
      for (int i = 0; i <= 2 * C; ++i) w[i] = wp[i];
#pragma unroll
      for (int i = 0; i < 2 * C; ++i) out[r * 2 * C + i] = __funnelshift_r(w[i], w[i + 1], 16);
    } else {
      const uint32_t* wp = reinterpret_cast<const uint32_t*>(slab + b0);
#pragma unroll
      for (int i = 0; i < 2 * C; ++i) out[r * 2 * C + i] = wp[i];
    }
#pragma unroll
    for (int i = 0; i < 2 * C; ++i) {
      const uint32_t m = ((2 * i >= lo && 2 * i < hi) ? 0xFFFFu : 0u) | ((2 * i + 1 >= lo && 2 * i + 1 < hi) ? 0xFFFF0000u : 0u);
      out[r * 2 * C + i] &= m;
    }
  }
  if (C < 4 && ones) out[8 * C] = 0x3F80u;
#pragma unroll
  for (int cc = 0; cc < 8; ++cc) *reinterpret_cast<uint4*>(tile + row * 128 + ((cc ^ (row & 7)) << 4)) = make_uint4(out[4 * cc], out[4 * cc + 1], out[4 * cc + 2], out[4 * cc + 3]);
}
__device__ __forceinline__ void edge_build_row(const TcEdgeParams& p, const uint8_t* slab, uint8_t* tile, int row, bool ones = false) {
  switch (p.C) { case 1: edge_build_row_c<1>(p, slab, tile, row, ones); break; case 2: edge_build_row_c<2>(p, slab, tile, row, ones); break;
                 case 3: edge_build_row_c<3>(p, slab, tile, row, ones); break; default: edge_build_row_c<4>(p, slab, tile, row, ones); break; }
}


__global__ void __launch_bounds__(128) tc_edge_conv_kernel(const TcEdgeParams p) { pdl_wait();
  extern __shared__ uint8_t smem_raw[];
  const uint32_t smem_base = (smem_u32(smem_raw) + 1023u) & ~1023u;
  uint8_t* sm = smem_raw + (smem_base - smem_u32(smem_raw));
  uint8_t* sA = sm; uint8_t* sB = sm + 16384; uint8_t* slab = sm + 24576;
  const int tid = threadIdx.x, warp = tid >> 5, lane = tid & 31;
  const int nb0 = blockIdx.y * 64, K = 16 * p.C;
  const int t_beg = blockIdx.x * p.tiles_per_cta, t_end = min(p.tiles_total, t_beg + p.tiles_per_cta);
  EdgeSlabRegs pre;
  if (t_beg < t_end) edge_fetch_slab(p, t_beg / p.tiles_y, (t_beg % p.tiles_y) * p.Ht, pre);
  {
    uint4 wv[4];
#pragma unroll
    for (int q = 0; q < 4; ++q) { const int i = tid + q * 128, o = i >> 3, cc = i & 7;
      wv[q] = cc < 2 * p.C ? __ldg(reinterpret_cast<const uint4*>(p.w + (size_t)(nb0 + o) * K) + cc) : make_uint4(0u, 0u, 0u, 0u); }
#pragma unroll
    for (int q = 0; q < 4; ++q) { const int i = tid + q * 128, o = i >> 3, cc = i & 7; *reinterpret_cast<uint4*>(sB + o * 128 + ((cc ^ (o & 7)) << 4)) = wv[q]; }
  }
  const bool has_bias = p.bias != nullptr;
  const int r0 = warp * 16 + (lane >> 2), cq = lane & 3;
  for (int t = t_beg; t < t_end; ++t) {
    const int n = t / p.tiles_y, oy0 = (t % p.tiles_y) * p.Ht;
    edge_store_slab(p, pre, slab);
    __syncthreads();
    if (t + 1 < t_end) edge_fetch_slab(p, (t + 1) / p.tiles_y, ((t + 1) % p.tiles_y) * p.Ht, pre);
    edge_build_row(p, slab, sA, tid);
    fence_proxy_async_smem();
    __syncthreads();
    float acc[2][32];
#pragma unroll
    for (int h = 0; h < 2; ++h)
#pragma unroll
      for (int j = 0; j < 32; ++j) acc[h][j] = 0.f;
    wg_fence();
    {
      const uint64_t bdesc = desc_kmajor_sw128(smem_base + 16384);
#pragma unroll
      for (int k = 0; k < 4; ++k)
#pragma unroll
        for (int h = 0; h < 2; ++h) wgmma_n64<0, 0>(acc[h], desc_kmajor_sw128(smem_base + h * 8192) + 2 * k, bdesc + 2 * k);
    }
    wg_commit();
    wg_wait<0>();
    __syncthreads();
#pragma unroll
    for (int h = 0; h < 2; ++h)
#pragma unroll
      for (int i = 0; i < 2; ++i) {
        const int row = h * 64 + r0 + 8 * i;
#pragma unroll
        for (int j = 0; j < 8; ++j) {
          const int col = j * 8 + 2 * cq;
          float a = acc[h][4 * j + 2 * i], b = acc[h][4 * j + 2 * i + 1];
          if (has_bias) { a += p.bias[nb0 + col]; b += p.bias[nb0 + col + 1]; }
          __nv_bfloat162 v = __floats2bfloat162_rn(act_fwd(p.act, a, p.alpha), act_fwd(p.act, b, p.alpha));
          *reinterpret_cast<__nv_bfloat162*>(sA + row * 128 + ((j ^ (row & 7)) << 4) + cq * 4) = v;
        }
      }
    __syncthreads();
// ... 263 lines not shown
```

gan_deeplearning4j_b200/engine.py:

```python
from __future__ import annotations

import copy
import ctypes as C
import math
from typing import Dict, List, Optional, Sequence

import numpy as np

from . import _lib
from ._lib import GanConfig, LayerDesc, LrSchedule, NetConfig, check

LAYER_TYPES = {"conv2d": 0, "deconv2d": 1, "batchnorm": 2, "dense": 3, "activation": 4, "maxpool": 5, "upsample2d": 6,
               "output": 7, "loss": 8, "ff_to_cnn": 9, "cnn_to_ff": 10, "dropout": 11, "subsampling": 12, "global_pooling": 13,
               "cnn_loss": 14, "elementwise": 15, "merge": 16}
ELEMENTWISE_OPS = {"add": 0, "subtract": 1, "product": 2, "average": 3, "max": 4}
VERTEX_TYPES = ("elementwise", "merge")
POOLINGS = {"max": 0, "avg": 1, "sum": 2, "pnorm": 3}
GLOBAL_PNORM_DEFAULT = 2
ACTS = {"identity": 0, "tanh": 1, "sigmoid": 2, "relu": 3, "lrelu": 4, "elu": 5, "selu": 6, "softplus": 7, "softsign": 8, "hardtanh": 9,
        "hardsigmoid": 10, "relu6": 11, "swish": 12, "cube": 13, "rationaltanh": 14, "rectifiedtanh": 15, "thresholdedrelu": 16}
ACT_ALPHA_DEFAULTS = {"elu": 1.0, "thresholdedrelu": 1.0}
LOSSES = {"xent": 0, "mcxent": 1, "mse": 2, "l1": 3, "l2": 4, "mae": 5, "hinge": 6, "squared_hinge": 7, "wasserstein": 8}
UPDATERS = {"sgd": 0, "rmsprop": 1, "adam": 2, "noop": 3, "nesterovs": 4, "adagrad": 5, "adamax": 6, "nadam": 7, "amsgrad": 8, "adadelta": 9}
NO_LR_UPDATERS = ("noop", "adadelta")
# ... 421 lines not shown
                continue
            sp[dropout_value_key(sp)] = copy.deepcopy(schedule) if schedule is not None else self.dropout_constants[sp["name"]]
            if layer is not None:
                break

    def dropout_value(self, layer: str) -> float:
        v = C.c_float()
        check(self.lib.b2g_net_get_dropout_value(self.h, layer.encode(), C.byref(v)))
        return v.value

    def learning_rate(self, layer: str) -> float:
        v = C.c_float()
        check(self.lib.b2g_net_get_learning_rate(self.h, layer.encode(), C.byref(v)))
        return v.value

    def epoch(self) -> int:
        v = C.c_int64()
        check(self.lib.b2g_net_get_epoch(self.h, C.byref(v)))
        return v.value

    def set_epoch(self, epoch: int):
        check(self.lib.b2g_net_set_epoch(self.h, int(epoch)))

    def set_grad_allreduce(self, enabled: bool):
        check(self.lib.b2g_net_set_grad_allreduce(self.h, int(enabled)))

    def set_sync_bn(self, enabled: bool):
        check(self.lib.b2g_net_set_sync_bn(self.h, int(enabled)))

    def set_grad_payload_bf16(self, enabled: bool):
        check(self.lib.b2g_net_set_grad_payload_bf16(self.h, int(enabled)))

    def enable_p2p_allreduce(self) -> bool:
        out = C.c_int32(0)
        check(self.lib.b2g_net_enable_p2p_allreduce(self.h, C.byref(out)))
        return bool(out.value)

    def average_parameters(self):
        check(self.lib.b2g_net_average_parameters(self.h))

    def iteration(self) -> int:
        v = C.c_int64()
        check(self.lib.b2g_net_get_iteration(self.h, C.byref(v)))
        return v.value

    def set_iteration(self, it: int):
        check(self.lib.b2g_net_set_iteration(self.h, int(it)))

    def dropout_pass(self) -> int:
        v = C.c_int64()
        check(self.lib.b2g_net_get_dropout_pass(self.h, C.byref(v)))
        return v.value

    def set_dropout_pass(self, p: int):
        check(self.lib.b2g_net_set_dropout_pass(self.h, int(p)))

    def simt_gemm_calls(self) -> int:
        v = C.c_uint64()
        check(self.lib.b2g_net_simt_gemm_calls(self.h, C.byref(v)))
        return v.value

    def time_hbm_kernels(self, rows: int, channels: int, iters: int = 10):
        ms = np.zeros(3, np.float32)
        check(self.lib.b2g_test_hbm_kernels(self.h, rows, channels, iters, _fp(ms)))
        return [float(v) for v in ms]

    def weight_operand(self, layer: int, which: int, size: int) -> np.ndarray:
        out = np.empty(size, np.float32)
        check(self.lib.b2g_test_net_shadow(self.h, layer, which, _fp(out), out.size))
        return out

    def input_gradient(self, batch: int) -> np.ndarray:
        out = np.empty((batch, int(np.prod(self.input_shape))), np.float32)
        check(self.lib.b2g_net_get_input_gradient(self.h, batch, _fp(out)))
        return out

    def close(self):
        if self.h:
            self.lib.b2g_net_destroy(self.h)
            self.h = None


class Gan:

    def __init__(self, gen: Net, dis: Net, fake_bn_train: bool = False, use_cuda_graph: bool = True):
        self.gen, self.dis, self.lib = gen, dis, gen.lib
        cfg = GanConfig(int(fake_bn_train), int(use_cuda_graph))
        h = C.c_void_p()
        check(self.lib.b2g_gan_create(gen.h, dis.h, C.byref(cfg), C.byref(h)))
        self.h = h

    def _args(self, x_real, z_d, z_g, y_real, y_fake, y_gen):
        x = _f32(x_real)
        n, oe = x.shape[0], self.dis.out_elems
        ys = []
        for name, y in (("y_real", y_real), ("y_fake", y_fake), ("y_gen", y_gen)):
            y = _f32(y).reshape(n, -1)
            if y.shape[1] == 1 and oe > 1:
                y = np.ascontiguousarray(np.broadcast_to(y, (n, oe)))
            if y.shape[1] != oe:
                raise ValueError(f"{name}: {y.shape[1]} labels per example; the discriminator has {oe} outputs per example (or pass one per image)")
            ys.append(y)
        return [x, _f32(z_d), _f32(z_g)] + ys

    def step(self, x_real, z_d, z_g, y_real, y_fake, y_gen):
        a = self._args(x_real, z_d, z_g, y_real, y_fake, y_gen)
        losses = np.zeros(3, np.float32)
        check(self.lib.b2g_gan_step(self.h, *[_fp(v) for v in a], a[0].shape[0], _fp(losses)))
        return losses

    def step_ptr(self, ptrs, batch: int, losses: np.ndarray):
        args = [C.cast(C.c_void_p(p), C.POINTER(C.c_float)) for p in ptrs]
        check(self.lib.b2g_gan_step(self.h, *args, batch, _fp(losses)))

    def upload(self, x_real, z_d, z_g, y_real, y_fake, y_gen):
        a = self._args(x_real, z_d, z_g, y_real, y_fake, y_gen)
        check(self.lib.b2g_gan_upload(self.h, *[_fp(v) for v in a], a[0].shape[0]))
        self.gen.ctx.sync()

    def step_resident(self, batch: int):
        check(self.lib.b2g_gan_step_resident(self.h, batch))

    def losses(self) -> np.ndarray:
        out = np.zeros(3, np.float32)
        check(self.lib.b2g_gan_read_losses(self.h, _fp(out)))
        return out

    def last_step_ms(self) -> float:
        v = C.c_float()
        check(self.lib.b2g_gan_last_step_ms(self.h, C.byref(v)))
        return v.value

    def close(self):
        if self.h:
            self.lib.b2g_gan_destroy(self.h)
            self.h = None


def test_conv(ctx: Context, kind: int, impl: int, precision: int, geom: Dict[str, int], a, b, out_size: int, iters: int = 1):
    g = _lib.ConvGeom(**geom)
    a, b = _f32(a).ravel(), _f32(b).ravel()
    out = np.empty(out_size, np.float32)
    ms = C.c_float()
    check(ctx.lib.b2g_test_conv(ctx.h, kind, impl, precision, C.byref(g), _fp(a), _fp(b), _fp(out), iters, C.byref(ms)))
    return out, ms.value


EPI_PLAIN, EPI_STATS, EPI_BNBWD, EPI_ACTBWD = 0, 1, 2, 3


def test_conv_ex(ctx: Context, kind: int, geom: Dict[str, int], a, b, out_size: int, *, epi: int = 0, act: str = "identity", alpha: float = 0.0,
                 bias=None, scale=None, groups: int = 1, aux=None, aux2=None, iters: int = 1, impl: int = 1, bn: int = 0, max_ctas: int = 0,
                 poison: bool = False, w_mn: bool = False, per_tap: bool = False, info: Optional[dict] = None, defer: bool = False, db=None,
                 precision: int = BF16, param_offset: int = 0, splits: int = 0):
    g = _lib.ConvGeom(**geom)
    a, b = _f32(a).ravel(), _f32(b).ravel()
    out = np.empty(out_size, np.float32)
    oc = geom["o"] if kind == 0 else geom["c"]
    o = _lib.TestConvOpts()
    o.epi, o.act, o.alpha, o.groups = epi, ACTS[act], alpha, groups
    o.bn, o.max_ctas, o.poison, o.w_mn, o.per_tap, o.defer = bn, max_ctas, int(poison), int(w_mn), int(per_tap), int(defer)
    o.param_offset, o.splits = param_offset, splits
    if db is not None:
        assert db.dtype == np.float32 and db.flags.c_contiguous
        o.db = _fp(db)
    keep = []
    for name, v in (("bias", bias), ("scale", scale), ("aux", aux), ("aux2", aux2)):
        if v is not None:
            arr = _f32(v).ravel(); keep.append(arr); setattr(o, name, _fp(arr))
    stats = None
    if epi in (EPI_STATS, EPI_BNBWD):
        stats = np.zeros((groups, 2, oc), np.float64); o.stats = stats.ctypes.data_as(C.POINTER(C.c_double))
    ms = C.c_float()
    check(ctx.lib.b2g_test_conv_ex(ctx.h, kind, impl, precision, C.byref(g), _fp(a), _fp(b), _fp(out), iters, C.byref(ms), C.byref(o)))
    if info is not None:
        info["slab"], info["splits"] = bool(o.slab), o.splits
    return out, stats, o.kernel.decode(), ms.value


def test_bn(ctx: Context, precision: int, path: int, x, eps_out, gamma, beta, run_mean, run_var, *, act: str = "identity", alpha: float = 0.0,
            eps: float = 1e-5, decay: float = 0.9, g_gamma=None, g_beta=None, want_param_grads: bool = True):
    x, e = _f32(x), _f32(eps_out)
    groups, rows, ch = x.shape
    par = [_f32(v).ravel() for v in (gamma, beta, run_mean, run_var)]
    r = {k: np.empty(x.shape, np.float32) for k in ("y", "eps_in")}
    r["g_gamma"] = _f32(np.zeros(ch) if g_gamma is None else g_gamma).copy()
    r["g_beta"] = _f32(np.zeros(ch) if g_beta is None else g_beta).copy()
    r.update({k: np.empty(ch, np.float32) for k in ("g_mean", "g_var")})
    r.update({k: np.empty((groups, ch), np.float32) for k in ("mean", "invstd")})
    check(ctx.lib.b2g_test_bn(ctx.h, precision, path, groups, rows, ch, _fp(x), _fp(e), *[_fp(v) for v in par], ACTS[act], alpha, eps, decay,
                              int(want_param_grads), *[_fp(r[k]) for k in ("y", "eps_in", "g_gamma", "g_beta", "g_mean", "g_var", "mean", "invstd")]))
    return r


def test_dropout_kind(ctx: Context, precision: int, kind: str, x, dy, value: float, *, seed: int = 666, layer: int = 0, rank: int = 0, pass_: int = 0):
    x, e = _f32(x), _f32(dy)
    rows = x.shape[0]
    h, w, c = (x.shape[1:] if x.ndim == 4 else (1, 1, int(np.prod(x.shape[1:]))))
    y, dx = np.empty_like(x), np.empty_like(x)
    check(ctx.lib.b2g_test_dropout_kind(ctx.h, precision, DROPOUT_KINDS[kind][0], seed, layer, rank, pass_, rows, h, w, c, value, _fp(x), _fp(e), _fp(y), _fp(dx)))
    return y, dx


def test_dropout(ctx: Context, precision: int, x, dy, p: float, *, seed: int = 666, layer: int = 0, rank: int = 0, pass_: int = 0):
    x, e = _f32(x), _f32(dy)
    rows = x.shape[0]
    h, w, c = (x.shape[1:] if x.ndim == 4 else (1, 1, int(np.prod(x.shape[1:]))))
    y, dx = np.empty_like(x), np.empty_like(x)
    check(ctx.lib.b2g_test_dropout(ctx.h, precision, seed, layer, rank, pass_, rows, h, w, c, p, _fp(x), _fp(e), _fp(y), _fp(dx)))
    return y, dx


EW_OPS = {"reduce_splits": 0, "reduce_multi": 1, "colsum": 2, "xent": 3, "softmax_xent": 4, "act_fwd": 5, "act_bwd": 6, "maxpool": 7,
          "upsample": 8, "sumsq": 9, "loss": 10, "act_ext_fwd": 11, "act_ext_bwd": 12,
          "cnn_xent": 13, "cnn_softmax_xent": 14, "vertex_fwd": 15, "vertex_bwd": 16, "merge_fwd": 17, "merge_bwd": 18, "skip_add": 19}


def test_ew(ctx: Context, precision: int, op: str, in0, in1=None, out_sizes=(0, 0, 0), *, act: str = "identity", jobs=None, segments=None,
            loss: str = "xent", **opts):
    o = _lib.TestEwOpts()
    o.op, o.act, o.loss = EW_OPS[op], ELEMENTWISE_OPS[act] if op in ("vertex_fwd", "vertex_bwd") else ACTS[act], LOSSES[loss]
    for k, v in opts.items():
        setattr(o, k, int(v) if isinstance(v, bool) else v)
    keep = []
    if jobs is not None:
        arr = (_lib.EwReduceJob * len(jobs))(*[_lib.EwReduceJob(j["n"], j["stride"], j["src_off"], j["dst_off"], j["splits"], 0) for j in jobs])
        o.n_jobs, o.jobs = len(jobs), arr
        keep.append(arr)
    if segments is not None:
        so, sl, sc = (np.ascontiguousarray(segments[0], np.int64), np.ascontiguousarray(segments[1], np.int64), _f32(segments[2]))
        keep += [so, sl, sc]
        o.n_seg = len(so)
        o.seg_off, o.seg_len, o.seg_coef = so.ctypes.data_as(C.POINTER(C.c_int64)), sl.ctypes.data_as(C.POINTER(C.c_int64)), _fp(sc)
    ins = [None if v is None else _f32(v).ravel() for v in (in0, in1)]
    outs = [np.empty(k, np.float32) if k else None for k in out_sizes]
    ptr = lambda a: None if a is None else _fp(a)
    check(ctx.lib.b2g_test_ew(ctx.h, precision, C.byref(o), *[ptr(a) for a in ins], *[ptr(a) for a in outs]))
    info = {"kernel": o.kernel.decode(), "sumsq": o.sumsq, "wide": [o.jobs[i].wide for i in range(o.n_jobs)] if jobs is not None else []}
    return outs, info


POOL_TEST_OPS = {"pool2d": 0, "global_pool": 1}


def test_pool(ctx: Context, precision: int, op: str, in0, in1, out_sizes=(0, 0, 0), *, pooling: str = "max", pnorm: float = 2.0, **opts):
    o = _lib.TestPoolOpts()
    o.op, o.pool, o.pnorm = POOL_TEST_OPS[op], POOLINGS[pooling], float(pnorm)
    for k, v in opts.items():
        setattr(o, k, int(v))
    ins = [_f32(v).ravel() for v in (in0, in1)]
    outs = [np.empty(k, np.float32) if k else None for k in out_sizes]
    ptr = lambda a: None if a is None else _fp(a)
    check(ctx.lib.b2g_test_pool(ctx.h, precision, C.byref(o), *[ptr(a) for a in ins], *[ptr(a) for a in outs]))
    return outs, {"kernel": o.kernel.decode(), "splits": o.splits}
```

include/b200gan.h:

```cpp
#ifndef B200GAN_H
#define B200GAN_H

#include <stddef.h>
#include <stdint.h>

#ifdef __cplusplus
extern "C" {
#endif

#define B2G_VERSION 101
#define B2G_NAME_LEN 64

typedef struct b2g_ctx b2g_ctx;
typedef struct b2g_net b2g_net;
typedef struct b2g_gan b2g_gan;

typedef enum {
  B2G_OK = 0,
  B2G_ERR_ARG = -1,
  B2G_ERR_SHAPE = -2,
  B2G_ERR_CUDA = -3,
  B2G_ERR_NCCL = -4,
  B2G_ERR_OOM = -5,
  B2G_ERR_UNSUPPORTED = -6,
// ... 44 lines not shown

typedef enum { B2G_PREC_FP32 = 0, B2G_PREC_BF16 = 1 } b2g_precision;
typedef enum {
  B2G_LOSS_XENT = 0, B2G_LOSS_MCXENT = 1, B2G_LOSS_MSE = 2, B2G_LOSS_L1 = 3, B2G_LOSS_L2 = 4, B2G_LOSS_MAE = 5, B2G_LOSS_HINGE = 6,
  B2G_LOSS_SQUARED_HINGE = 7, B2G_LOSS_WASSERSTEIN = 8
} b2g_loss;

typedef struct {
  int32_t type;
  char name[B2G_NAME_LEN];
  int32_t n_in, n_out;
  int32_t k_h, k_w, s_h, s_w, p_h, p_w;
  int32_t has_bias;
  int32_t act;
  float act_alpha;
  int32_t updater;
  float lr, beta1, beta2, eps;
  float l2;
  float bn_decay, bn_eps;
  int32_t pre_h, pre_w, pre_c;
  int32_t loss;
  int32_t frozen;
} b2g_layer_desc;

typedef struct {
  int32_t in_h, in_w, in_c;
  int32_t max_batch;
  int32_t precision;
  float grad_clip;
  float xent_clip_eps;
  int32_t bn_groups;
  uint64_t seed;
} b2g_net_config;

int32_t b2g_version(void);
int32_t b2g_ctx_create(int32_t device, b2g_ctx** out);
int32_t b2g_ctx_destroy(b2g_ctx* ctx);
const char* b2g_last_error(void);
int32_t b2g_sync(b2g_ctx* ctx);
int32_t b2g_launch_count(b2g_ctx* ctx, uint64_t* out);
int32_t b2g_timer_start(b2g_ctx* ctx);
int32_t b2g_timer_stop_ms(b2g_ctx* ctx, float* ms);
int32_t b2g_flush_l2(b2g_ctx* ctx);
int32_t b2g_device_info(b2g_ctx* ctx, int32_t* sm_count, int32_t* cc_major, int32_t* cc_minor, uint64_t* mem_bytes);

int32_t b2g_net_create(b2g_ctx* ctx, const b2g_net_config* cfg, const b2g_layer_desc* layers, int32_t n_layers, b2g_net** out);
int32_t b2g_net_destroy(b2g_net* net);
int32_t b2g_net_num_params(b2g_net* net, int64_t* out);
int32_t b2g_net_output_size(b2g_net* net, int64_t* per_example);
int32_t b2g_net_layer_output_size(b2g_net* net, int32_t layer, int64_t* per_example);
int32_t b2g_net_set_param(b2g_net* net, const char* layer, const char* param, const float* host, int64_t n);
int32_t b2g_net_get_param(b2g_net* net, const char* layer, const char* param, float* host, int64_t n);
int32_t b2g_net_get_params(b2g_net* net, float* host, int64_t n);
int32_t b2g_net_set_params(b2g_net* net, const float* host, int64_t n);
int32_t b2g_net_get_gradients(b2g_net* net, float* host, int64_t n);
int32_t b2g_net_updater_state_size(b2g_net* net, int64_t* out);
int32_t b2g_net_get_updater_state(b2g_net* net, float* host, int64_t n);
int32_t b2g_net_set_updater_state(b2g_net* net, const float* host, int64_t n);
int32_t b2g_net_output(b2g_net* net, const float* x, int32_t batch, int32_t train, float* out);
int32_t b2g_net_get_activation(b2g_net* net, int32_t layer, int32_t batch, float* host);
int32_t b2g_net_compute_gradient_and_score(b2g_net* net, const float* x, const float* y, int32_t batch, float* score);
int32_t b2g_net_get_input_gradient(b2g_net* net, int32_t batch, float* host);
int32_t b2g_net_fit(b2g_net* net, const float* x, const float* y, int32_t batch, float* score);
int32_t b2g_net_get_iteration(b2g_net* net, int64_t* out);
int32_t b2g_net_set_iteration(b2g_net* net, int64_t iteration);
int32_t b2g_net_get_dropout_pass(b2g_net* net, int64_t* out);
int32_t b2g_net_set_dropout_pass(b2g_net* net, int64_t pass);
typedef enum {
  B2G_GN_NONE = 0, B2G_GN_RENORM_L2_LAYER = 1, B2G_GN_RENORM_L2_PARAM = 2, B2G_GN_CLIP_ELEMENTWISE = 3, B2G_GN_CLIP_L2_LAYER = 4, B2G_GN_CLIP_L2_PARAM = 5
} b2g_gradient_normalization;
int32_t b2g_net_set_gradient_normalization(b2g_net* net, int32_t mode, float threshold);
typedef enum {
  B2G_CONSTRAINT_MAX_NORM = 0, B2G_CONSTRAINT_MIN_MAX_NORM = 1, B2G_CONSTRAINT_UNIT_NORM = 2, B2G_CONSTRAINT_NON_NEGATIVE = 3
} b2g_constraint_kind;
typedef struct {
  int32_t kind;
  int32_t dims_mask;
  double max_norm, min_norm, rate;
} b2g_constraint;
int32_t b2g_net_set_constraints(b2g_net* net, const char* layer, const char* param, const b2g_constraint* list, int32_t n);
int32_t b2g_net_apply_constraints(b2g_net* net);
typedef enum {
  B2G_SCHED_NONE = 0, B2G_SCHED_EXPONENTIAL = 1, B2G_SCHED_INVERSE = 2, B2G_SCHED_SIGMOID = 3, B2G_SCHED_STEP = 4, B2G_SCHED_MAP = 5
} b2g_schedule_kind;
typedef enum { B2G_SCHED_ITERATION = 0, B2G_SCHED_EPOCH = 1 } b2g_schedule_type;
typedef struct {
  int32_t kind, type;
  double initial, gamma, power, step, decay_rate;
  int32_t n_map;
  const int32_t* map_keys;
  const double* map_values;
} b2g_lr_schedule;
int32_t b2g_net_set_lr_schedule(b2g_net* net, const char* layer, const b2g_lr_schedule* s);
int32_t b2g_net_get_learning_rate(b2g_net* net, const char* layer, float* out);
int32_t b2g_net_set_dropout_schedule(b2g_net* net, const char* layer, const b2g_lr_schedule* s);
int32_t b2g_net_get_dropout_value(b2g_net* net, const char* layer, float* out);
int32_t b2g_net_get_epoch(b2g_net* net, int64_t* out);
int32_t b2g_net_set_epoch(b2g_net* net, int64_t epoch);
int32_t b2g_net_simt_gemm_calls(b2g_net* net, uint64_t* out);

typedef struct {
  int32_t fake_bn_train;
  int32_t use_cuda_graph;
} b2g_gan_config;
int32_t b2g_gan_create(b2g_net* gen, b2g_net* dis, const b2g_gan_config* cfg, b2g_gan** out);
int32_t b2g_gan_destroy(b2g_gan* gan);
int32_t b2g_gan_step(b2g_gan* gan, const float* x_real, const float* z_d, const float* z_g,
                     const float* y_real, const float* y_fake, const float* y_gen, int32_t batch, float* losses);
int32_t b2g_gan_upload(b2g_gan* gan, const float* x_real, const float* z_d, const float* z_g,
                       const float* y_real, const float* y_fake, const float* y_gen, int32_t batch);
int32_t b2g_gan_step_resident(b2g_gan* gan, int32_t batch);
int32_t b2g_gan_read_losses(b2g_gan* gan, float* losses);
int32_t b2g_gan_last_step_ms(b2g_gan* gan, float* ms);

#define B2G_NCCL_ID_BYTES 128
int32_t b2g_comm_unique_id(void* id128);
int32_t b2g_ctx_comm_init(b2g_ctx* ctx, int32_t world, int32_t rank, const void* id128);
int32_t b2g_ctx_comm_destroy(b2g_ctx* ctx);
int32_t b2g_net_set_grad_allreduce(b2g_net* net, int32_t enabled);
int32_t b2g_net_average_parameters(b2g_net* net);
int32_t b2g_net_set_sync_bn(b2g_net* net, int32_t enabled);
int32_t b2g_net_set_grad_payload_bf16(b2g_net* net, int32_t enabled);
int32_t b2g_net_enable_p2p_allreduce(b2g_net* net, int32_t* enabled);
int32_t b2g_ctx_allreduce_test(b2g_ctx* ctx, float* host_inout, int64_t n);

typedef struct {
  int32_t n, h, w, c;
  int32_t oh, ow, o;
  int32_t kh, kw, sh, sw, ph, pw;
} b2g_conv_geom;
int32_t b2g_test_conv(b2g_ctx* ctx, int32_t kind, int32_t impl, int32_t precision, const b2g_conv_geom* g,
                      const float* x_or_dy, const float* w_or_x, float* out, int32_t iters, float* ms_per_iter);
typedef struct {
  int32_t epi;
  int32_t act; float alpha;
  const float* bias;
  const float* scale;
  int32_t groups;
  const float* aux;
  const float* aux2;
  double* stats;
  char kernel[64];
  int32_t bn;
  int32_t max_ctas;
  int32_t poison;
  int32_t w_mn;
  int32_t per_tap;
  int32_t slab;
  int32_t defer;
  float* db;
  int32_t param_offset;
  int32_t splits;
} b2g_test_conv_opts;
int32_t b2g_test_conv_ex(b2g_ctx* ctx, int32_t kind, int32_t impl, int32_t precision, const b2g_conv_geom* g,
                         const float* x_or_dy, const float* w_or_x, float* out, int32_t iters, float* ms_per_iter, b2g_test_conv_opts* opts);

int32_t b2g_test_hbm_kernels(b2g_net* net, int32_t rows, int32_t channels, int32_t iters, float* ms3);

int32_t b2g_test_bn(b2g_ctx* ctx, int32_t precision, int32_t path, int32_t groups, int32_t rows, int32_t C, const float* x, const float* eps_out,
                    const float* gamma, const float* beta, const float* run_mean, const float* run_var, int32_t act, float alpha, float eps, float decay,
                    int32_t want_param_grads, float* y, float* eps_in, float* g_gamma, float* g_beta, float* g_mean, float* g_var, float* mean, float* invstd);
int32_t b2g_test_net_shadow(b2g_net* net, int32_t layer, int32_t which, float* out, int64_t n);
int32_t b2g_test_dropout(b2g_ctx* ctx, int32_t precision, uint64_t seed, int32_t layer, int32_t rank, int64_t pass, int32_t rows, int32_t h, int32_t w,
                         int32_t c, float p, const float* x, const float* dy, float* y, float* dx);
int32_t b2g_test_dropout_kind(b2g_ctx* ctx, int32_t precision, int32_t kind, uint64_t seed, int32_t layer, int32_t rank, int64_t pass, int32_t rows,
                              int32_t h, int32_t w, int32_t c, float value, const float* x, const float* dy, float* y, float* dx);

typedef enum {
  B2G_EW_REDUCE_SPLITS = 0, B2G_EW_REDUCE_MULTI = 1, B2G_EW_COLSUM = 2, B2G_EW_XENT = 3, B2G_EW_SOFTMAX_XENT = 4,
  B2G_EW_ACT_FWD = 5, B2G_EW_ACT_BWD = 6, B2G_EW_MAXPOOL = 7, B2G_EW_UPSAMPLE = 8, B2G_EW_SUMSQ = 9, B2G_EW_LOSS = 10,
  B2G_EW_ACT_EXT_FWD = 11, B2G_EW_ACT_EXT_BWD = 12, B2G_EW_CNN_XENT = 13, B2G_EW_CNN_SOFTMAX_XENT = 14,
  B2G_EW_VERTEX_FWD = 15, B2G_EW_VERTEX_BWD = 16, B2G_EW_MERGE_FWD = 17, B2G_EW_MERGE_BWD = 18, B2G_EW_SKIP_ADD = 19
} b2g_ew_op;
typedef struct {
  int64_t n, stride, src_off, dst_off;
  int32_t splits;
  int32_t wide;
} b2g_ew_reduce_job;
typedef struct {
  int32_t op;
  int64_t n;
  int32_t rows, cols;
  int32_t groups;
  int32_t splits; int64_t stride;
  int32_t N, H, W, C, KH, KW, SH, SW;
  int32_t act; float alpha;
  float clip_eps;
  int32_t offset;
  int32_t in_place;
  int32_t accumulate;
  int32_t poison;
  int32_t n_jobs; b2g_ew_reduce_job* jobs;
  int32_t n_seg; const int64_t* seg_off; const int64_t* seg_len; const float* seg_coef;
  double sumsq;
  char kernel[64];
  int32_t loss;
} b2g_test_ew_opts;
int32_t b2g_test_ew(b2g_ctx* ctx, int32_t precision, b2g_test_ew_opts* opts, const float* in0, const float* in1, float* out0, float* out1, float* out2);

typedef enum { B2G_TEST_POOL2D = 0, B2G_TEST_GLOBAL_POOL = 1 } b2g_test_pool_op;
typedef struct {
  int32_t op;
  int32_t pool;
  float pnorm;
  int32_t N, H, W, C, KH, KW, SH, SW, PH, PW;
  int32_t offset;
  int32_t poison;
  char kernel[64];
  int32_t splits;
} b2g_test_pool_opts;
int32_t b2g_test_pool(b2g_ctx* ctx, int32_t precision, b2g_test_pool_opts* opts, const float* in0, const float* in1, float* out0, float* out1, float* out2);

#ifdef __cplusplus
}
#endif
#endif
```

Baseline: 92090.

## Add 256-row two-consumer-warpgroup tensor-core conv kernel for k4s2p1 layers

Adds a warp-specialized tensor-core conv kernel. One producer warp feeds two 128-row consumer warpgroups through a shared TMA ring, so each B tile is reused across 256 output rows, and it uses setmaxnreg to rebalance registers. The epilogue is split into chunk and fold helpers and staged through a padded shared-memory chunk buffer per warpgroup. The new kernel is picked automatically for 4x4 stride-2 layers with BN=64, no slab, and enough K-blocks and work items. It trades fewer stages and larger register and shared-memory pressure for better B reuse and fewer CTAs.

Result: faster. 93160, median of 6 (+1.2%).

```diff
diff --git a/gan_deeplearning4j_b200/_lib.py b/gan_deeplearning4j_b200/_lib.py
--- a/gan_deeplearning4j_b200/_lib.py
+++ b/gan_deeplearning4j_b200/_lib.py
@@ -136,6 +136,7 @@
     "b2g_ctx_allreduce_test": (_i32, [_vp, _fp, _i64]),
     "b2g_test_conv": (_i32, [_vp, _i32, _i32, _i32, C.POINTER(ConvGeom), _fp, _fp, _fp, _i32, _fp]),
     "b2g_test_hbm_kernels": (_i32, [_vp, _i32, _i32, _i32, _fp]),
+    "b2g_test_tc_rows": (_i32, [_i32]),
     "b2g_test_conv_ex": (_i32, [_vp, _i32, _i32, _i32, C.POINTER(ConvGeom), _fp, _fp, _fp, _i32, _fp, C.POINTER(TestConvOpts)]),
     "b2g_test_bn": (_i32, [_vp, _i32, _i32, _i32, _i32, _i32, _fp, _fp, _fp, _fp, _fp, _fp, _i32, C.c_float, C.c_float, C.c_float,
                            _i32, _fp, _fp, _fp, _fp, _fp, _fp, _fp, _fp]),
diff --git a/gan_deeplearning4j_b200/csrc/engine.cu b/gan_deeplearning4j_b200/csrc/engine.cu
--- a/gan_deeplearning4j_b200/csrc/engine.cu
+++ b/gan_deeplearning4j_b200/csrc/engine.cu
@@ -1729,6 +1729,10 @@
 };
 static constexpr int ik(int impl, int kind) { return 3 * impl + kind; }
 
+extern "C" int32_t b2g_test_tc_rows(int32_t rows) {
+  if (rows != 0 && rows != 128 && rows != 256) return -1;
+  const int last = g_tc_last_rows; g_tc_test_rows = rows; return last;
+}
 extern "C" int32_t b2g_test_conv_ex(b2g_ctx* c, int32_t kind, int32_t impl, int32_t precision, const b2g_conv_geom* gg, const float* a_host, const float* b_host, float* out, int32_t iters, float* ms_per_iter,
                                     b2g_test_conv_opts* opt) {
   if (!c || !gg || !a_host || !b_host || !out) return fail(B2G_ERR_ARG, "null");
@@ -1796,7 +1800,7 @@
   ReduceList rl{}; ReduceList* prl = o.defer ? &rl : nullptr;
   cudaEvent_t e0, e1; B2(m.event(&e0)); B2(m.event(&e1));
   int reps = iters < 1 ? 1 : iters; int rc = 0, db_written = 0;
-  g_tc_last_kernel = ""; g_tc_last_slab = false; g_tc_last_splits = 0; g_gemm_last_kernel = ""; g_gemm_last_splits = 0;
+  g_tc_last_kernel = ""; g_tc_last_slab = false; g_tc_last_rows = 0; g_tc_last_splits = 0; g_gemm_last_kernel = ""; g_gemm_last_splits = 0;
   TcTestSchedule schedule(o.bn, o.max_ctas, o.per_tap != 0, force_splits);
   for (int it = -1; it < reps; ++it) {
     if (it == 0) CU(cudaEventRecord(e0, s));
diff --git a/gan_deeplearning4j_b200/csrc/kernels.h b/gan_deeplearning4j_b200/csrc/kernels.h
--- a/gan_deeplearning4j_b200/csrc/kernels.h
+++ b/gan_deeplearning4j_b200/csrc/kernels.h
@@ -236,6 +236,7 @@
 extern int g_tc_test_per_tap;
 extern bool g_tc_last_slab;
 extern int g_tc_test_splits, g_tc_last_splits;
+extern int g_tc_test_rows, g_tc_last_rows;
 enum { EPI_PLAIN = 0, EPI_STATS = 1, EPI_BNBWD = 2, EPI_ACTBWD = 3 };
 struct TcEpi {
   int mode;
diff --git a/gan_deeplearning4j_b200/csrc/kernels_tc.cu b/gan_deeplearning4j_b200/csrc/kernels_tc.cu
--- a/gan_deeplearning4j_b200/csrc/kernels_tc.cu
+++ b/gan_deeplearning4j_b200/csrc/kernels_tc.cu
@@ -163,17 +163,17 @@
 }
 __device__ __forceinline__ void warp_colsum32(float (&a)[32], int lane) { warp_colsum_level<16>(a, lane); }
 
+__device__ __forceinline__ void epi_row_offsets(size_t roff, int lane, size_t (&roff_i)[4]) {
+#pragma unroll
+  for (int i = 0; i < 4; ++i) roff_i[i] = __shfl_sync(0xffffffffu, (unsigned long long)roff, i * 8 + (lane >> 2)) + (lane & 3) * 8;
+}
 template <int BN, int EPI, bool AFFINE>
-__device__ __forceinline__ void epi_tile(const TcConvParams& p, const float* srow, size_t roff, int nb0, int group, float* sst, uint4* stg, int q, int lane, int ep_tid,
-                                         int c_beg, int c_end) {
+__device__ __forceinline__ void epi_chunk(const TcConvParams& p, const float* src, const size_t (&roff_i)[4], int nb0, float* sst, uint4* stg, int q, int lane,
+                                          int c0) {
   constexpr bool stats = EPI == EPI_STATS || EPI == EPI_BNBWD;
   const bool has_bias = p.bias != nullptr;
   const int sub = lane >> 2, cq = lane & 3, sx = (lane >> 1) & 3;
-  size_t roff_i[4];
-#pragma unroll
-  for (int i = 0; i < 4; ++i) roff_i[i] = __shfl_sync(0xffffffffu, (unsigned long long)roff, i * 8 + sub) + cq * 8;
-#pragma unroll 1
-  for (int c0 = c_beg; c0 < c_end; c0 += 32) {
+  {
     uint32_t v[32];
     uint4 gy[4], gz[4], ax[4], az[4];
     if constexpr (EPI >= EPI_BNBWD) {
@@ -201,7 +201,7 @@
       __syncwarp();
     }
 #pragma unroll
-    for (int j = 0; j < 8; ++j) { const uint4 t = reinterpret_cast<const uint4*>(srow + c0)[j]; v[4 * j] = t.x; v[4 * j + 1] = t.y; v[4 * j + 2] = t.z; v[4 * j + 3] = t.w; }
+    for (int j = 0; j < 8; ++j) { const uint4 t = reinterpret_cast<const uint4*>(src)[j]; v[4 * j] = t.x; v[4 * j + 1] = t.y; v[4 * j + 2] = t.z; v[4 * j + 3] = t.w; }
     float o[32], s2[32];
     if constexpr (EPI == EPI_BNBWD) {
       const __nv_bfloat162* yb = reinterpret_cast<const __nv_bfloat162*>(ax);
@@ -269,15 +269,27 @@
       sst[(q * 2 + 1) * BN + c0 + lane] = s2[0];
     }
   }
-  if constexpr (stats) {
+}
+template <int BN>
+__device__ __forceinline__ void epi_fold(const TcConvParams& p, const float* sst, int group, int nb0, int tid, int nthreads) {
+  for (int col = tid; col < BN; col += nthreads) {
+#pragma unroll
+    for (int st = 0; st < 2; ++st) {
+      const float s = ((sst[(0 * 2 + st) * BN + col] + sst[(1 * 2 + st) * BN + col]) + sst[(2 * 2 + st) * BN + col]) + sst[(3 * 2 + st) * BN + col];
+      sacc_add(p.acc + (size_t)(group * 2 + st) * 2 * p.OC, (size_t)p.OC, (size_t)(nb0 + col), s);
+    }
+  }
+}
+template <int BN, int EPI, bool AFFINE>
+__device__ __forceinline__ void epi_tile(const TcConvParams& p, const float* srow, size_t roff, int nb0, int group, float* sst, uint4* stg, int q, int lane, int ep_tid,
+                                         int c_beg, int c_end) {
+  size_t roff_i[4];
+  epi_row_offsets(roff, lane, roff_i);
+#pragma unroll 1
+  for (int c0 = c_beg; c0 < c_end; c0 += 32) epi_chunk<BN, EPI, AFFINE>(p, srow + c0, roff_i, nb0, sst, stg, q, lane, c0);
+  if constexpr (EPI == EPI_STATS || EPI == EPI_BNBWD) {
     epi_bar_sync();
-    for (int col = ep_tid; col < BN; col += 256) {
-#pragma unroll
-      for (int st = 0; st < 2; ++st) {
-        const float s = ((sst[(0 * 2 + st) * BN + col] + sst[(1 * 2 + st) * BN + col]) + sst[(2 * 2 + st) * BN + col]) + sst[(3 * 2 + st) * BN + col];
-        sacc_add(p.acc + (size_t)(group * 2 + st) * 2 * p.OC, (size_t)p.OC, (size_t)(nb0 + col), s);
-      }
-    }
+    epi_fold<BN>(p, sst, group, nb0, ep_tid, 256);
   }
 }
 
@@ -489,10 +501,163 @@
   }
 }
 
+static constexpr int TC_CONV256_THREADS = 384;
+static constexpr int CHUNK_PITCH = 36;
+template <int BN, int STAGES, int EPI, bool SLAB>
+struct Tc256Smem {
+  static constexpr int A_HALF = (SLAB ? SLAB_ROWS : 128) * 128;
+  static constexpr int A_BYTES = 2 * A_HALF;
+  static constexpr int B_BYTES = (SLAB ? 2 : 1) * BN * 128;
+  static constexpr int STAGE_BYTES = A_BYTES + B_BYTES;
+  static constexpr int RING_BYTES = STAGES * STAGE_BYTES;
+  static constexpr int CHUNK_BYTES = 128 * CHUNK_PITCH * 4;
+  static constexpr int CHUNK_OFF = RING_BYTES;
+  static constexpr int BAR_OFF = CHUNK_OFF + 2 * CHUNK_BYTES;
+  static constexpr int STAT_OFF = BAR_OFF + 256;
+  static constexpr int STAT_WG = (EPI == EPI_STATS || EPI == EPI_BNBWD) ? 4 * 2 * BN * 4 : 0;
+  static constexpr int STG_OFF = STAT_OFF + 2 * STAT_WG;
+  static constexpr int TOTAL = STG_OFF + 8 * 2048 + 1024;
+  static_assert(STAGE_BYTES % 1024 == 0, "ring stages must keep the SW128 tiles 1024-byte aligned");
+  static_assert(TOTAL <= 227 * 1024, "one CTA per SM must fit the shared memory of an sm_90 SM");
+};
+struct Tc256Regs {
+  static constexpr int LAUNCH = 168, PRODUCER = 40, MMA = 232;
+  static_assert(PRODUCER + 2 * MMA <= 3 * LAUNCH, "setmaxnreg budget exceeds the launch allocation");
+};
+__device__ __forceinline__ void wg_bar_sync(int h) { asm volatile("bar.sync %0, 128;" ::"r"(1 + h) : "memory"); }
+
+template <int BN, int STAGES, int EPI, bool AFFINE, bool SLAB>
+__global__ void __launch_bounds__(TC_CONV256_THREADS, 1) tc_conv256_kernel(const __grid_constant__ CUtensorMap tmA, const __grid_constant__ CUtensorMap tmB, const TcConvParams p) {
+  using S = Tc256Smem<BN, STAGES, EPI, SLAB>;
+  using R = Tc256Regs;
+  constexpr int NB = BN / 64;
+  extern __shared__ uint8_t smem_raw[];
+  const uint32_t smem_base = (smem_u32(smem_raw) + 1023u) & ~1023u;
+  uint8_t* smem_gen = smem_raw + (smem_base - smem_u32(smem_raw));
+  const uint32_t bar_full = smem_base + S::BAR_OFF;
+  const uint32_t bar_empty = bar_full + 8 * STAGES;
+  const int warp = threadIdx.x >> 5, lane = threadIdx.x & 31;
+  const int num_kb = p.taps_h * p.taps_w * p.chunks;
+  const int pairs_m = p.tiles_m / 2;
+  const int items = pairs_m * p.tiles_n * p.phases;
+  auto item_coords = [&](int t, int& nb0, int& phase, int& mt0) {
+    const int r = t / pairs_m;
+    mt0 = 2 * (t % pairs_m); nb0 = (r % p.tiles_n) * BN; phase = r / p.tiles_n;
+  };
+  auto tile_origin = [&](int mt, int& n0, int& y0) { if (p.Nt > 1) { n0 = mt * p.Nt; y0 = 0; } else { n0 = mt / p.tiles_y; y0 = (mt % p.tiles_y) * p.Ht; } };
+
+  if (threadIdx.x == 0) {
+    prefetch_map(&tmA); prefetch_map(&tmB);
+    for (int s = 0; s < STAGES; ++s) { mbar_init(bar_full + 8 * s, 1); mbar_init(bar_empty + 8 * s, 8); }
+    fence_mbar_init();
+  }
+  __syncthreads();
+  pdl_wait();
+
+  if (warp >= 8) {
+    setmaxnreg_dec<R::PRODUCER>();
+    if (warp == 8) {
+      int s = 0; uint32_t ph = 0;
+      for (int t = blockIdx.x; t < items; t += gridDim.x) {
+        int nb0, phase, mt0; item_coords(t, nb0, phase, mt0);
+        const int py = phase >> 1, px = phase & 1;
+        int n0[2], ybase[2];
+#pragma unroll
+        for (int h = 0; h < 2; ++h) { int y0; tile_origin(mt0 + h, n0[h], y0); ybase[h] = p.mode == 0 ? y0 * p.SH : y0; }
+        int ch = 0, ta = 0, tb = 0;
+        int ax, dy_, wtap, wtap2 = 0;
+        auto coords = [&]() { if constexpr (SLAB) slab_coords(p, ta, tb, py, px, ax, dy_, wtap, wtap2); else tap_coords(p, ta, tb, py, px, ax, dy_, wtap); };
+        coords();
+        for (int kb = 0; kb < num_kb; ++kb) {
+          mbar_wait(bar_empty + 8 * s, ph ^ 1);
+          if (elect_one_sync()) {
+            const uint32_t st = smem_base + s * S::STAGE_BYTES;
+            mbar_expect_tx(bar_full + 8 * s, SLAB ? 2 * p.slab_bytes + S::B_BYTES : S::STAGE_BYTES);
+#pragma unroll
+            for (int h = 0; h < 2; ++h) tma_load_4d(st + h * S::A_HALF, &tmA, bar_full + 8 * s, ch * 64, ax, ybase[h] + dy_, n0[h]);
+            load_b_tile<BN>(p, &tmB, st + S::A_BYTES, bar_full + 8 * s, ch, wtap, nb0);
+            if constexpr (SLAB) load_b_tile<BN>(p, &tmB, st + S::A_BYTES + BN * 128, bar_full + 8 * s, ch, wtap2, nb0);
+          }
+          __syncwarp();
+          if (++s == STAGES) { s = 0; ph ^= 1; }
+          if (++ch == p.chunks) { ch = 0; if (++tb == p.taps_w) { tb = 0; ++ta; } coords(); }
+        }
+      }
+    }
+  } else {
+    setmaxnreg_inc<R::MMA>();
+    const int h = warp >> 2, q = warp & 3;
+    const int r0 = q * 16 + (lane >> 2), row = q * 32 + lane;
+    const int img = row / (p.Ht * p.Wt), rem = row % (p.Ht * p.Wt), yy = rem / p.Wt, xx = rem % p.Wt;
+    float* chunk = reinterpret_cast<float*>(smem_gen + S::CHUNK_OFF + h * S::CHUNK_BYTES);
+    float* sst = reinterpret_cast<float*>(smem_gen + S::STAT_OFF + h * S::STAT_WG);
+    uint4* stg = reinterpret_cast<uint4*>(smem_gen + S::STG_OFF) + warp * 128;
+    int s = 0; uint32_t ph = 0;
+    for (int t = blockIdx.x; t < items; t += gridDim.x) {
+      float acc[2][NB][32];
+#pragma unroll
+      for (int mb = 0; mb < 2; ++mb)
+#pragma unroll
+        for (int nb = 0; nb < NB; ++nb)
+#pragma unroll
+          for (int j = 0; j < 32; ++j) acc[mb][nb][j] = 0.f;
+      int prev = -1;
+      for (int kb = 0; kb < num_kb; ++kb) {
+        mbar_wait(bar_full + 8 * s, ph);
+        wg_fence();
+        const uint32_t st = smem_base + s * S::STAGE_BYTES, a = st + h * S::A_HALF;
+        if constexpr (SLAB) {
+#pragma unroll
+          for (int mb = 0; mb < 2; ++mb) mma_kblock<BN, NB, 32>(acc[mb], a + mb * p.a_wg_bytes, st + S::A_BYTES, p.b_mn);
+#pragma unroll
+          for (int mb = 0; mb < 2; ++mb) mma_kblock<BN, NB, 32>(acc[mb], a + mb * p.a_wg_bytes + p.a_tap_bytes, st + S::A_BYTES + BN * 128, p.b_mn);
+        } else {
+#pragma unroll
+          for (int mb = 0; mb < 2; ++mb) mma_kblock<BN, NB, 32>(acc[mb], a + mb * 8192, st + S::A_BYTES, p.b_mn);
+        }
+        wg_commit();
+        wg_wait<1>();
+        if (prev >= 0 && lane == 0) mbar_arrive(bar_empty + 8 * prev);
+        prev = s;
+        if (++s == STAGES) { s = 0; ph ^= 1; }
+      }
+      wg_wait<0>();
+      if (lane == 0) mbar_arrive(bar_empty + 8 * prev);
+
+      int nb0, phase, mt0, n0, y0; item_coords(t, nb0, phase, mt0); tile_origin(mt0 + h, n0, y0);
+      const int py = phase >> 1, px = phase & 1;
+      const int n = n0 + img, gy = y0 + yy, gx = xx;
+      const size_t pix = p.mode == 0 ? ((size_t)n * p.outH + gy) * p.outW + gx : ((size_t)n * p.outH + 2 * gy + py) * p.outW + 2 * gx + px;
+      size_t roff_i[4];
+      epi_row_offsets(pix * p.OC + nb0, lane, roff_i);
+#pragma unroll
+      for (int c = 0; c < BN / 32; ++c) {
+        wg_bar_sync(h);
+#pragma unroll
+        for (int mb = 0; mb < 2; ++mb)
+#pragma unroll
+          for (int jj = 0; jj < 4; ++jj) {
+            const int j = (c & 1) * 4 + jj, col = jj * 8 + 2 * (lane & 3), rr = mb * 64 + r0;
+            const float* d = acc[mb][c >> 1];
+            *reinterpret_cast<float2*>(chunk + rr * CHUNK_PITCH + col) = make_float2(d[4 * j], d[4 * j + 1]);
+            *reinterpret_cast<float2*>(chunk + (rr + 8) * CHUNK_PITCH + col) = make_float2(d[4 * j + 2], d[4 * j + 3]);
+          }
+        wg_bar_sync(h);
+        epi_chunk<BN, EPI, AFFINE>(p, chunk + row * CHUNK_PITCH, roff_i, nb0, sst, stg, q, lane, 32 * c);
+      }
+      if constexpr (EPI == EPI_STATS || EPI == EPI_BNBWD) {
+        wg_bar_sync(h);
+        epi_fold<BN>(p, sst, p.imgs_per_group > 0 ? n0 / p.imgs_per_group : 0, nb0, threadIdx.x & 127, 128);
+      }
+    }
+  }
+}
+
 const char* g_tc_last_kernel = "";
 bool g_tc_last_slab = false;
 int g_tc_test_bn = 0, g_tc_test_max_ctas = 0, g_tc_test_per_tap = 0, g_tc_test_splits = 0;
 int g_tc_last_splits = 0;
+int g_tc_test_rows = 0, g_tc_last_rows = 0;
 static int tc_device() { int dev = 0; cudaGetDevice(&dev); return dev < 0 || dev >= 64 ? 0 : dev; }
 #define TC_SET_SMEM_ONCE(kernel, bytes)                                                                                            \
   do { static bool set_[64] = {}; const int d_ = tc_device();                                                                       \
@@ -546,13 +711,43 @@
   }
   return (p.scale && p.bias) ? launch_conv_e<BN, STAGES, EPI_PLAIN, true, false, SLAB>(tmA, tmB, p, s) : launch_conv_e<BN, STAGES, EPI_PLAIN, false, false, SLAB>(tmA, tmB, p, s);
 }
-static int dispatch_conv(int BN, bool slab, const CUtensorMap& tmA, const CUtensorMap& tmB, const TcConvParams& p, cudaStream_t s) {
-  switch (BN * 2 + slab) {
+template <int BN, int STAGES, int EPI, bool AFFINE, bool SLAB>
+static int launch_conv256_e(const CUtensorMap& tmA, const CUtensorMap& tmB, const TcConvParams& p, cudaStream_t s) {
+  using S = Tc256Smem<BN, STAGES, EPI, SLAB>;
+  TC_SET_SMEM_ONCE((tc_conv256_kernel<BN, STAGES, EPI, AFFINE, SLAB>), S::TOTAL);
+  const long items = (long)(p.tiles_m / 2) * p.tiles_n * p.phases;
+  const unsigned grid = (unsigned)std::min<long>(items, g_tc_test_max_ctas > 0 ? g_tc_test_max_ctas : device_sm_count());
+  launch_pdl(tc_conv256_kernel<BN, STAGES, EPI, AFFINE, SLAB>, dim3(grid), dim3(TC_CONV256_THREADS), (size_t)(S::TOTAL), s, tmA, tmB, p);
+  LAUNCHED();
+  return cudaPeekAtLastError() == cudaSuccess ? 0 : -3;
+}
+template <int BN, int STAGES, bool SLAB>
+static int launch_conv256(const CUtensorMap& tmA, const CUtensorMap& tmB, const TcConvParams& p, cudaStream_t s, const char* name) {
+  g_tc_last_kernel = name; g_tc_last_slab = SLAB;
+  switch (p.epi) {
+    case EPI_STATS: return launch_conv256_e<BN, STAGES, EPI_STATS, false, SLAB>(tmA, tmB, p, s);
+    case EPI_BNBWD: return launch_conv256_e<BN, STAGES, EPI_BNBWD, false, SLAB>(tmA, tmB, p, s);
+    case EPI_ACTBWD: return launch_conv256_e<BN, STAGES, EPI_ACTBWD, false, SLAB>(tmA, tmB, p, s);
+  }
+  return (p.scale && p.bias) ? launch_conv256_e<BN, STAGES, EPI_PLAIN, true, SLAB>(tmA, tmB, p, s) : launch_conv256_e<BN, STAGES, EPI_PLAIN, false, SLAB>(tmA, tmB, p, s);
+}
+static int dispatch_conv(int BN, bool slab, int rows, const CUtensorMap& tmA, const CUtensorMap& tmB, const TcConvParams& p, cudaStream_t s) {
+  g_tc_last_rows = rows;
+  switch ((rows == 256) * 1000 + BN * 2 + slab) {
     case 128: return launch_conv<64, 4, false>(tmA, tmB, p, s, "tc_conv_kernel<64,4>");
     case 256: return launch_conv<128, 4, false>(tmA, tmB, p, s, "tc_conv_kernel<128,4>");
     case 129: return launch_conv<64, 4, true>(tmA, tmB, p, s, "tc_conv_kernel<64,4>");
+    case 1128: return launch_conv256<64, 4, false>(tmA, tmB, p, s, "tc_conv_kernel<64,4>");
+    case 1256: return launch_conv256<128, 3, false>(tmA, tmB, p, s, "tc_conv_kernel<128,4>");
+    case 1129: return launch_conv256<64, 3, true>(tmA, tmB, p, s, "tc_conv_kernel<64,4>");
   }
   return -4;
+}
+static int pick_rows(const TcConvParams& p, int BN, bool slab, bool k4s2p1) {
+  const bool can = p.tiles_m % 2 == 0;
+  if (g_tc_test_rows) return g_tc_test_rows == 256 && !can ? 0 : g_tc_test_rows;
+  const long items = (long)(p.tiles_m / 2) * p.tiles_n * p.phases;
+  return can && k4s2p1 && BN == 64 && !slab && p.taps_h * p.taps_w * p.chunks >= 32 && 8 * items >= 7L * device_sm_count() ? 256 : 128;
 }
 static bool slab_tile(const TcConvParams& p, int BN) {
   if (g_tc_test_per_tap || BN != 64 || p.Wt % 8) return false;
@@ -591,15 +786,17 @@
   fill_epi(p, bias, act, alpha, epi);
   const bool slab = is_k4s2p1_geom(g) && !w_mn && slab_tile(p, BN);
   if (slab) set_slab(p);
+  p.tiles_m = g.N * g.OH * g.OW / 128; p.tiles_n = g.O / BN; p.phases = 1;
+  const int rows = pick_rows(p, BN, slab, is_k4s2p1_geom(g) && !w_mn);
+  if (!rows) return -1;
   CUtensorMap tmA, tmB;
   cuuint64_t dims[4] = {(cuuint64_t)g.C, (cuuint64_t)g.W, (cuuint64_t)g.H, (cuuint64_t)g.N};
   cuuint64_t strides[3] = {(cuuint64_t)g.C * 2, (cuuint64_t)g.W * g.C * 2, (cuuint64_t)g.H * g.W * g.C * 2};
   cuuint32_t box[4] = {64, (cuuint32_t)(p.Wt * g.SW), (cuuint32_t)((p.Ht + slab) * g.SH), (cuuint32_t)p.Nt};
   cuuint32_t es[4] = {1, (cuuint32_t)g.SW, (cuuint32_t)g.SH, 1};
   if (make_map_bf16(&tmA, x, 4, dims, strides, box, es)) return -1;
-  p.tiles_m = g.N * g.OH * g.OW / 128; p.tiles_n = g.O / BN; p.phases = 1;
   if (w_mn ? weight_map(&tmB, w, g.C, 1, g.O, 64) : weight_map(&tmB, w, g.O, g.KH * g.KW, g.C, BN)) return -1;
-  return dispatch_conv(BN, slab, tmA, tmB, p, s);
+  return dispatch_conv(BN, slab, rows, tmA, tmB, p, s);
 }
 
 int k_tc_dgrad(const ConvGeom& g, const __nv_bfloat16* dy, const __nv_bfloat16* w, const float* bias, __nv_bfloat16* dx, int act, float alpha, cudaStream_t s, const TcEpi* epi) {
@@ -611,6 +808,9 @@
   fill_epi(p, bias, act, alpha, epi);
   const bool slab = slab_tile(p, BN);
   if (slab) set_slab(p);
+  p.tiles_m = g.N * g.OH * g.OW / 128; p.tiles_n = g.C / BN; p.phases = 4;
+  const int rows = pick_rows(p, BN, slab, true);
+  if (!rows) return -1;
   CUtensorMap tmA, tmB;
   cuuint64_t dims[4] = {(cuuint64_t)g.O, (cuuint64_t)g.OW, (cuuint64_t)g.OH, (cuuint64_t)g.N};
   cuuint64_t strides[3] = {(cuuint64_t)g.O * 2, (cuuint64_t)g.OW * g.O * 2, (cuuint64_t)g.OH * g.OW * g.O * 2};
@@ -618,8 +818,7 @@
   cuuint32_t es[4] = {1, 1, 1, 1};
   if (weight_map(&tmB, w, g.O, 16, g.C, 64)) return -1;
   if (make_map_bf16(&tmA, dy, 4, dims, strides, box, es)) return -1;
-  p.tiles_m = g.N * g.OH * g.OW / 128; p.tiles_n = g.C / BN; p.phases = 4;
-  return dispatch_conv(BN, slab, tmA, tmB, p, s);
+  return dispatch_conv(BN, slab, rows, tmA, tmB, p, s);
 }
 
 bool tc_deconv_ps_shape(const ConvGeom& g) { return is_k4s2p1_geom(g) && g.C >= 1 && g.C <= 4 && g.O % 64 == 0; }
diff --git a/gan_deeplearning4j_b200/engine.py b/gan_deeplearning4j_b200/engine.py
--- a/gan_deeplearning4j_b200/engine.py
+++ b/gan_deeplearning4j_b200/engine.py
@@ -597,7 +597,7 @@
 def test_conv_ex(ctx: Context, kind: int, geom: Dict[str, int], a, b, out_size: int, *, epi: int = 0, act: str = "identity", alpha: float = 0.0,
                  bias=None, scale=None, groups: int = 1, aux=None, aux2=None, iters: int = 1, impl: int = 1, bn: int = 0, max_ctas: int = 0,
                  poison: bool = False, w_mn: bool = False, per_tap: bool = False, info: Optional[dict] = None, defer: bool = False, db=None,
-                 precision: int = BF16, param_offset: int = 0, splits: int = 0):
+                 precision: int = BF16, param_offset: int = 0, splits: int = 0, rows: int = 0):
     g = _lib.ConvGeom(**geom)
     a, b = _f32(a).ravel(), _f32(b).ravel()
     out = np.empty(out_size, np.float32)
@@ -617,9 +617,14 @@
     if epi in (EPI_STATS, EPI_BNBWD):
         stats = np.zeros((groups, 2, oc), np.float64); o.stats = stats.ctypes.data_as(C.POINTER(C.c_double))
     ms = C.c_float()
-    check(ctx.lib.b2g_test_conv_ex(ctx.h, kind, impl, precision, C.byref(g), _fp(a), _fp(b), _fp(out), iters, C.byref(ms), C.byref(o)))
+    if ctx.lib.b2g_test_tc_rows(rows) < 0:
+        raise ValueError(f"rows {rows}: the work item is 128 or 256 rows (0: production choice)")
+    try:
+        check(ctx.lib.b2g_test_conv_ex(ctx.h, kind, impl, precision, C.byref(g), _fp(a), _fp(b), _fp(out), iters, C.byref(ms), C.byref(o)))
+    finally:
+        ran_rows = ctx.lib.b2g_test_tc_rows(0)
     if info is not None:
-        info["slab"], info["splits"] = bool(o.slab), o.splits
+        info["slab"], info["rows"], info["splits"] = bool(o.slab), ran_rows, o.splits
     return out, stats, o.kernel.decode(), ms.value
 
 
diff --git a/include/b200gan.h b/include/b200gan.h
--- a/include/b200gan.h
+++ b/include/b200gan.h
@@ -220,6 +220,7 @@
   int32_t param_offset;
   int32_t splits;
 } b2g_test_conv_opts;
+int32_t b2g_test_tc_rows(int32_t rows);
 int32_t b2g_test_conv_ex(b2g_ctx* ctx, int32_t kind, int32_t impl, int32_t precision, const b2g_conv_geom* g,
                          const float* x_or_dy, const float* w_or_x, float* out, int32_t iters, float* ms_per_iter, b2g_test_conv_opts* opts);
 
```
